# zfwangDP/X2-GNN

Measured on AMD Instinct MI355X. Metric: molecules/sec (fwd+bwd) on QM9 U0, batch=128, 1/2/4/8 MI355X, higher is better.
Workload: dtype fp32; 1 GPU; xgnn_poly U0 train step (config.json: L=4, D=128, H=16, sbf 7x6), S160, fwd+loss+bwd+allreduce+clip+Adam+EMA; per_gpu_batch=128, global_batch=128, line_nodes_per_gpu=21058, triplets_per_gpu=194060, parallelism=dp1, hip_graph=True

## Files before the change

include/x2g.h:

```cpp
#ifndef X2G_H
#define X2G_H

#include <stddef.h>
#include <stdint.h>

#ifdef __cplusplus
extern "C" {
#endif

#define X2G_OK 0
#define X2G_EINVAL 1001
#define X2G_EUNSUPPORTED 1002
#define X2G_EWORKSPACE 1003

#define X2G_EDGE_NONE 0
#define X2G_EDGE_PER_TRIPLET 1
#define X2G_EDGE_PER_DST 2

int x2g_abi_version(void);
const char* x2g_status_string(int status);


int x2g_csr_rowptr(const int32_t* keys, int64_t n, int64_t n_seg, int32_t* rowptr, void* stream);

// ... 230 lines not shown
int x2g_smooth_l1_mean_fwd_grad(const float* pred, const float* target, int64_t n, float beta, float* out,
                                float* dpred_unit, void* stream);


size_t x2g_linear_wgrad_workspace(int64_t rows, int32_t out_features, int32_t in_features);


#define X2G_ACCUM_WGRAD 1
#define X2G_DEFER_SLAB_SUM 2

typedef struct {
  const float* part_w;
  const float* part_b;
  float* dw;
  float* db;
  int64_t n_w;
  int32_t n_b;
  int32_t splits;
  int32_t ld;
  int32_t cols;
} x2g_slab_job;

int x2g_slab_sum_batch(const x2g_slab_job* jobs, int32_t njobs, int32_t accum, void* stream);

#define X2G_GATE_MAX_JOBS 8
typedef struct {
  const float* x;
  const float* w;
  const float* b;
  float* out;
  const float* g;
  float* dx;
  const float* dx_add;
  float* dw;
  float* db;
} x2g_gate_job;
int x2g_rbf_pool_fwd_batch(const x2g_gate_job* jobs, int32_t n_jobs, const float* rbf, const int32_t* rowptr,
                           int64_t n_seg, int32_t D, int32_t R, void* stream);
size_t x2g_rbf_gate_bwd_batch_workspace(int64_t rows, int32_t D, int32_t R, int32_t n_jobs);
int x2g_rbf_gate_bwd_batch(const x2g_gate_job* jobs, int32_t n_jobs, const int32_t* owner, const float* rbf,
                           int64_t rows, int32_t D, int32_t R, float* drbf, int flags, x2g_slab_job* slab_jobs,
                           void* workspace, size_t workspace_bytes, void* stream);

int32_t x2g_linear_wgrad_splits(int64_t rows, int32_t out_features, int32_t in_features);
int32_t x2g_dense_bwd_splits(int64_t rows, int32_t in_features, int32_t out_features);
int64_t x2g_dense_bwd_slab_offset(int64_t rows, int32_t in_features, int32_t out_features);

int x2g_linear_wgrad_ex(const float* dy, const float* x, int64_t rows, int32_t out_features,
                        int32_t in_features, float* dw, float* db, int flags, void* workspace,
                        size_t workspace_bytes, void* stream);

#define X2G_ACT_NONE 0
#define X2G_ACT_SILU 1

int x2g_dense_fwd(const float* x, const float* w, const float* b, int64_t rows, int32_t in_features,
                  int32_t out_features, int act, const float* res, float* y, float* z, void* stream);

size_t x2g_dense_bwd_workspace(int64_t rows, int32_t in_features, int32_t out_features);

int x2g_dense_bwd(const float* dy, const float* z, int act, const float* x, const float* w, int64_t rows,
                  int32_t in_features, int32_t out_features, float* dx, float* dw, float* db, void* workspace,
                  size_t workspace_bytes, void* stream);

int x2g_dense_bwd_ex(const float* dy, const float* z, int act, const float* x, const float* w, int64_t rows,
                     int32_t in_features, int32_t out_features, float* dx, const float* dx_add, float* dw,
                     float* db, int flags, void* workspace, size_t workspace_bytes, void* stream);

int x2g_residual_fwd(const float* x, const float* w0, const float* b0, const float* w1, const float* b1,
                     int64_t rows, int32_t dim, float* h, float* z0, float* z1, float* y, void* stream);

#define X2G_MAX_GROUPS 8

typedef struct {
  const float* x;
  const float* w;
  const float* b;
  const float* res;
  float* y;
  float* z;
} x2g_dense_fwd_group;

typedef struct {
  const float* dy;
  const float* z;
  const float* x;
  const float* w;
  float* dx;
  const float* dx_add;
  float* dw;
  float* db;
} x2g_dense_bwd_group;

int x2g_dense_fwd_batched(const x2g_dense_fwd_group* groups, int32_t num_groups, int64_t rows,
                          int32_t in_features, int32_t out_features, int act, void* stream);

int x2g_dense_bwd_batched(const x2g_dense_bwd_group* groups, int32_t num_groups, int64_t rows,
                          int32_t in_features, int32_t out_features, int act, int flags, void* workspace,
                          size_t workspace_bytes, void* stream);

typedef struct {
  const float* h;
  const float* w;
  const float* b;
  float* dh;
  float* dw;
  float* db;
} x2g_head_group;

int x2g_readout_head_fwd(const x2g_head_group* groups, int32_t num_groups, int64_t rows, int32_t dim, float* out,
                         void* stream);
size_t x2g_readout_head_bwd_workspace(int64_t rows, int32_t dim, int32_t num_groups);
int32_t x2g_readout_head_bwd_splits(int64_t rows);
int x2g_readout_head_bwd(const float* dout, const x2g_head_group* groups, int32_t num_groups, int64_t rows,
                         int32_t dim, int flags, void* workspace, size_t workspace_bytes, void* stream);

int x2g_readout_head_pool_fwd(const x2g_head_group* groups, int32_t num_groups, int64_t rows, int32_t dim,
                              const int32_t* seg_rowptr, int64_t num_segments, float* out_seg, void* stream);
int x2g_readout_head_pool_bwd(const float* dout_seg, const int32_t* seg_rowptr, int64_t num_segments,
                              const x2g_head_group* groups, int32_t num_groups, int64_t rows, int32_t dim, int flags,
                              void* workspace, size_t workspace_bytes, void* stream);


#define X2G_OPT_LR 0
#define X2G_OPT_BETA1 1
#define X2G_OPT_BETA2 2
#define X2G_OPT_EPS 3
#define X2G_OPT_MAX_NORM 4
#define X2G_OPT_EMA_DECAY 5
#define X2G_OPT_STEP 6
#define X2G_OPT_NORM 7
#define X2G_OPT_CLIP 8
#define X2G_OPT_STEP_SIZE 9
#define X2G_OPT_BC2_SQRT 10
#define X2G_OPT_WARMUP 11
#define X2G_OPT_DECAY_STEPS 12
#define X2G_OPT_DECAY_RATE 13
#define X2G_OPT_BASE_LR 14
#define X2G_OPT_STAIRCASE 15

size_t x2g_optimizer_workspace(int64_t n);

int x2g_clip_adam_ema(float* params, const float* grads, float* exp_avg, float* exp_avg_sq, float* ema,
                      int64_t n, float* scalars, void* workspace, size_t workspace_bytes, void* stream);
#define X2G_OPT_ZERO_GRADS 1
int x2g_clip_adam_ema_ex(float* params, float* grads, float* exp_avg, float* exp_avg_sq, float* ema, int64_t n,
                         float* scalars, int flags, void* workspace, size_t workspace_bytes, void* stream);

#define X2G_CHAIN_MAX_STAGES 8
#define X2G_CHAIN_SILU 1
#define X2G_CHAIN_HOLD 2
#define X2G_CHAIN_RES_HELD 4
#define X2G_CHAIN_RES_EXT 8
#define X2G_CHAIN_RES_ACCUM 16

typedef struct {
  const float* w;
  const float* b;
  float* z;
  float* y;
  float* wt;
  int32_t flags;
} x2g_chain_stage;

int x2g_chain_fwd(const float* x, const float* res_ext, const x2g_chain_stage* stages, int32_t n_stages,
                  int64_t rows, int32_t dim, float* in_t, void* stream);

int x2g_chain_fwd_ln(const float* x, const float* row_stats, const int32_t* seg_rowptr, int64_t num_segments,
                     float eps, float* x_norm, float* seg_mean, float* seg_rstd, const float* res_ext,
                     const x2g_chain_stage* stages, int32_t n_stages, int64_t rows, int32_t dim, float* in_t,
                     void* stream);

#define X2G_CHAIN_MAX_JOBS 8
typedef struct {
  const float* x;
  const float* res_ext;
  const x2g_chain_stage* stages;
  float* in_t;
} x2g_chain_fwd_job;
int x2g_chain_fwd_batch(const x2g_chain_fwd_job* jobs, int32_t num_jobs, int32_t n_stages, int64_t rows, int32_t dim,
                        void* stream);

int64_t x2g_chain_t_floats(int64_t rows, int32_t dim);

typedef struct {
  const float* w;
  const float* wt;
  const float* z;
  float* dz;
  int32_t flags;
} x2g_chain_bwd_stage;

int x2g_chain_bwd(const float* dy, const float* dy_add, const x2g_chain_bwd_stage* stages, int32_t n_stages,
                  int64_t rows, int32_t dim, float* dx, float* d_res_ext, float* dz_t, void* stream);
int x2g_chain_bwd_ln(const float* dy, const float* dy_add, const x2g_chain_bwd_stage* stages, int32_t n_stages,
                     int64_t rows, int32_t dim, float* dx, float* d_res_ext, float* dz_t, const float* x_norm,
                     float* row_gstats, void* stream);

typedef struct {
  const float* dy;
  const float* dy_add;
  const x2g_chain_bwd_stage* stages;
  float* dx;
  float* d_res_ext;
  float* dz_t;
} x2g_chain_bwd_job;
int x2g_chain_bwd_batch(const x2g_chain_bwd_job* jobs, int32_t num_jobs, int32_t n_stages, int64_t rows, int32_t dim,
                        void* stream);

size_t x2g_chain_wgrad_workspace(int64_t rows, int32_t dim, int32_t n_stages);
int x2g_chain_wgrad(const float* in_t, const float* dz_t, int32_t n_stages, int64_t rows, int32_t dim,
                    float* const* dw, float* const* db, int flags, void* workspace, size_t workspace_bytes,
                    void* stream);

typedef struct {
  const float* dy;
  const float* x;
  float* dw;
  float* db;
} x2g_wgrad_job;

size_t x2g_wgrad_batched_workspace(int64_t rows, int32_t dim, int32_t num_jobs);
int32_t x2g_wgrad_batched_splits(int64_t rows, int32_t dim, int32_t num_jobs);
int x2g_wgrad_batched(const x2g_wgrad_job* jobs, int32_t num_jobs, int64_t rows, int32_t dim, int flags,
                      void* workspace, size_t workspace_bytes, void* stream);

typedef struct {
  const float* w;
  const float* b;
  float* out;
  float* wt;
} x2g_proj;

int x2g_conv_proj_fwd(const float* x, const float* rbf, int32_t rbf_dim, const float* w_rbf, const x2g_proj* proj,
                      int64_t rows, int32_t dim, float* x_t, float* xs_t, void* stream);

typedef struct {
  const float* g;
  const float* w;
  const float* wt;
  float* g_t;
} x2g_proj_grad;

int32_t x2g_conv_proj_bwd_gate_splits(int64_t rows);
size_t x2g_conv_proj_bwd_gate_workspace(int64_t rows, int32_t rbf_dim);
int x2g_conv_proj_bwd_gate(const x2g_proj_grad* grads, int64_t rows, int32_t dim, const float* x, const float* rbf,
                           int32_t rbf_dim, const float* w_rbf, float* dx, const float* dx_add, float* drbf,
                           float* dw_rbf, int flags, void* workspace, size_t workspace_bytes, void* stream);

typedef struct {
  const float* dy_t;
  const float* x_t;
  float* dw;
  float* db;
  int32_t ld;
  int32_t cols;
} x2g_tiled_job;

#define X2G_TILED_MAX_JOBS 64
size_t x2g_tiled_wgrad_flat_workspace(int64_t rows, int32_t dim, int32_t num_jobs);
int x2g_tiled_wgrad_flat(const x2g_tiled_job* jobs, int32_t num_jobs, int64_t rows, int32_t dim, int flags,
                         x2g_slab_job* slab_jobs, void* workspace, size_t workspace_bytes, void* stream);
size_t x2g_tiled_wgrad_flat_rows_workspace(const int64_t* job_rows, int32_t num_jobs, int32_t dim);
int x2g_tiled_wgrad_flat_rows(const x2g_tiled_job* jobs, const int64_t* job_rows, int32_t num_jobs, int32_t dim,
                              int flags, x2g_slab_job* slab_jobs, void* workspace, size_t workspace_bytes,
                              void* stream);

size_t x2g_tiled_wgrad_workspace(int64_t rows, int32_t dim, int32_t num_jobs);
int x2g_tiled_wgrad(const x2g_tiled_job* jobs, int32_t num_jobs, int64_t rows, int32_t dim, int flags,
                    void* workspace, size_t workspace_bytes, void* stream);

#define X2G_TABLE_MAX_STAGES 8

typedef struct {
  const float* w;
  const float* b;
  int32_t parent;
  int32_t act;
  float* z;
  float* y;
} x2g_table_stage;

int x2g_table_chain_fwd(const float* x, int64_t rows, int32_t dim, const x2g_table_stage* stages, int32_t n_stages,
                        void* stream);

typedef struct {
  const float* w;
  const float* in;
  const float* z;
  const float* dy;
  float* dw;
  float* db;
  int32_t parent;
  int32_t act;
  int32_t accum;
} x2g_table_bwd_stage;

size_t x2g_table_chain_bwd_workspace(int32_t n_stages);
int x2g_table_chain_bwd_ex(const x2g_table_bwd_stage* stages, int32_t n_stages, int64_t rows, int32_t dim, float* dx,
                           void* workspace, size_t workspace_bytes, void* stream);

int x2g_feat_fwd(const float* x, const float* env, int64_t rows, int32_t in_dim, const float* w1, const float* b1,
                 const float* w2, const float* b2, float* y, float* xs_t, float* z1_t, float* y1_t, float* z2_t,
                 void* stream);

int x2g_feat_bwd(const float* dy, const float* z2_t, const float* z1_t, const float* w2, int64_t rows, float* dz2_t,
                 float* dz1_t, void* stream);

#ifdef __cplusplus
}
#endif

#endif
```

x2-gnn_amd/csrc/chain.hip:

```cpp
#include <math.h>

#include <type_traits>

#include "common.hpp"

namespace x2g {
namespace {

typedef float f4 __attribute__((ext_vector_type(4)));

constexpr int kCD = 128;
constexpr int kCWaves = 8;
constexpr int kCThreads = kCWaves * 64;

struct ChainFwdArgs {
  const float* x;
  const float* res;
  float* in_t;
  int64_t tf;
  int64_t R;
  int n;
  x2g_chain_stage st[X2G_CHAIN_MAX_STAGES];
};

// ... 378 lines not shown
  }
  float cnt = 0.f;
#pragma unroll
  for (int j = 0; j < kPW; ++j) cnt += (lane + 64 * j <= ln.G && pk[j] <= r0) ? 1.f : 0.f;
  for (int64_t k = lane + 64 * kPW; k <= ln.G; k += 64) cnt += ln.ptr[k] <= r0 ? 1.f : 0.f;
  const int64_t m0 = static_cast<int64_t>(wave64_sum(cnt)) - 1;
  auto ptr_at = [&](int64_t k) -> int {
    if (k >= 64 * kPW) return uniform(ln.ptr[k]);
    const int l = static_cast<int>(k & 63);
    switch (k >> 6) {
      case 0: return lane_bcast(pk[0], l);
      case 1: return lane_bcast(pk[1], l);
      case 2: return lane_bcast(pk[2], l);
      default: return lane_bcast(pk[3], l);
    }
  };
  constexpr int kSW = 4;
  for (int64_t m = m0 > 0 ? m0 : 0; m < ln.G; ++m) {
    const int p0 = ptr_at(m), p1 = ptr_at(m + 1);
    if (p0 >= r0 + nrows) break;
    if (p1 - p0 <= kLongMol) continue;
    const float n = static_cast<float>(p1 - p0);
    constexpr int kU = 4;
    float s = 0.f;
    for (int base = p0 + tid; base < p1; base += kU * kCThreads) {
      float v[kU];
#pragma unroll
      for (int u = 0; u < kU; ++u) {
        const int r = base + u * kCThreads;
        v[u] = r < p1 ? ln.stats[r].x : 0.f;
      }
#pragma unroll
      for (int u = 0; u < kU; ++u) s += v[u];
    }
    s = wave64_sum(s);
    if (lane == 0) red[w] = s;
    __syncthreads();
    float st = 0.f;
#pragma unroll
    for (int ww = 0; ww < kCWaves; ++ww) st += red[ww];
    const float mu = st / n;
    float q = 0.f;
    for (int base = p0 + tid; base < p1; base += kU * kCThreads) {
      float2 v[kU];
#pragma unroll
      for (int u = 0; u < kU; ++u) {
        const int r = base + u * kCThreads;
        v[u] = r < p1 ? ln.stats[r] : make_float2(mu, 0.f);
      }
#pragma unroll
      for (int u = 0; u < kU; ++u) {
        const float d = v[u].x - mu;
        q += fmaf(static_cast<float>(kCD) * d, d, v[u].y);
      }
    }
    q = wave64_sum(q);
    if (lane == 0) red[kCWaves + w] = q;
    __syncthreads();
    float qt = 0.f;
#pragma unroll
    for (int ww = 0; ww < kCWaves; ++ww) qt += red[kCWaves + ww];
    const float denom = sqrtf(qt / (n * static_cast<float>(kCD)) + ln.eps);
    const int lo = p0 > r0 ? p0 : r0, hi = p1 < r0 + nrows ? p1 : r0 + nrows;
    for (int r = lo + tid; r < hi; r += kCThreads) lnrow[r - r0] = make_float2(mu, denom);
    if (tid == 0 && p0 >= r0) {
      if (ln.mean) ln.mean[m] = mu;
      if (ln.rstd) ln.rstd[m] = 1.0f / denom;
    }
    __syncthreads();
  }
  for (int64_t m = (m0 > 0 ? m0 : 0) + w; m < ln.G; m += kCWaves) {
    const int p0 = ptr_at(m), p1 = ptr_at(m + 1);
    if (p0 >= r0 + nrows) break;
    if (p1 <= p0 || p1 - p0 > kLongMol) continue;
    const float n = static_cast<float>(p1 - p0);
    float2 sv[kSW];
#pragma unroll
    for (int j = 0; j < kSW; ++j) {
      const int r = p0 + lane + 64 * j;
      sv[j] = ln.stats[r < p1 ? r : p0];
    }
    float s = 0.f;
#pragma unroll
    for (int j = 0; j < kSW; ++j) s += p0 + lane + 64 * j < p1 ? sv[j].x : 0.f;
    for (int r = p0 + lane + 64 * kSW; r < p1; r += 64) s += ln.stats[r].x;
    const float mu = wave64_sum(s) / n;
    float q = 0.f;
#pragma unroll
    for (int j = 0; j < kSW; ++j) {
      const float d = sv[j].x - mu;
      q += p0 + lane + 64 * j < p1 ? fmaf(static_cast<float>(kCD) * d, d, sv[j].y) : 0.f;
    }
    for (int r = p0 + lane + 64 * kSW; r < p1; r += 64) {
      const float2 st = ln.stats[r];
      const float d = st.x - mu;
      q += fmaf(static_cast<float>(kCD) * d, d, st.y);
    }
    const float denom = sqrtf(wave64_sum(q) / (n * static_cast<float>(kCD)) + ln.eps);
    const int lo = p0 > r0 ? p0 : r0, hi = p1 < r0 + nrows ? p1 : r0 + nrows;
    for (int r = lo + lane; r < hi; r += 64) lnrow[r - r0] = make_float2(mu, denom);
    if (lane == 0 && p0 >= r0) {
      if (ln.mean) ln.mean[m] = mu;
      if (ln.rstd) ln.rstd[m] = 1.0f / denom;
    }
  }
  asm volatile("s_waitcnt vmcnt(0)" ::: "memory");
  __syncthreads();
#pragma unroll
  for (int u = 0; u < RB; ++u) {
    const int q = tid + kCThreads * u, r = q >> 5, c = q & 31;
    const bool ok = r < nrows;
    const float2 st = lnrow[ok ? r : 0];
    const f4 v = img[ipos(r, c)];
    f4 y;
#pragma unroll
    for (int e = 0; e < 4; ++e) y[e] = ok ? (v[e] - st.x) / st.y : 0.0f;
    img[ipos(r, c)] = y;
    if (ln.out && ok) *reinterpret_cast<f4*>(ln.out + (r0 + r) * kCD + 4 * c) = y;
  }
}

template <bool LN, int RB = kV2RB, bool TC = true>
__device__ __forceinline__ void chain_fwd_v4_run(const ChainFwdArgs& a, const ChainLn& ln) {
  static_assert(RB == 6 || RB == 3, "thirds of 2 or 1 row blocks");
  __shared__ f4 img0[RB * 16 * 32];
  __shared__ f4 img1[RB * 16 * 32];
  __shared__ f4 imgr[RB * 16 * 32];
  __shared__ float2 lnrow[LN ? RB * 16 : 1];
  __shared__ float lnred[LN ? 2 * kCWaves : 1];
  const int tid = threadIdx.x, lane = tid & 63, w = tid >> 6;
  const int rl = lane & 15, g = lane >> 4;
  const int64_t nblk = (a.R + 15) / 16, G = gridDim.x;
  const int64_t nch = (nblk + RB * G - 1) / (RB * G) * G;
  const int n = a.n;
  for (int64_t i = static_cast<int64_t>(blockIdx.x) * kCThreads + tid; i < static_cast<int64_t>(n) * kCD * kCD;
       i += G * kCThreads) {
    const int s = static_cast<int>(i / (kCD * kCD)), e = static_cast<int>(i % (kCD * kCD));
    if (a.st[s].wt) a.st[s].wt[e] = a.st[s].w[(e % kCD) * kCD + e / kCD];
  }
  for (int64_t ch = blockIdx.x; ch < nch; ch += G) {
    int r0, nrows;
    chunk_rows(ch, nch, nblk, a.R, r0, nrows);
    __syncthreads();
    if (LN)
      stage_rows_ln<RB>(img0, a.x, a.R, ln, lnrow, lnred, r0, nrows);
    else
      stage_rows<RB>(img0, a.x, nullptr, r0, nrows);
    if (a.res) stage_rows<RB>(imgr, a.res, nullptr, r0, nrows);
    f4 A[8], held[RB];
    load_slice<false>(a.st[0].w, w, rl, g, A);
#pragma unroll
    for (int rb = 0; rb < RB; ++rb) held[rb] = zero4();
    __syncthreads();
    if (a.in_t) {
      f4 xs[RB];
#pragma unroll
      for (int rb = 0; rb < RB; ++rb) xs[rb] = img0[ipos(16 * rb + rl, 4 * w + g)];
      store_t_slice(a.in_t, xs, r0, nrows, w, rl, g);
    }
    for (int s = 0; s < n; s += 2) {
      fwd4_stage<RB, TC>(a, s, img0, img1, imgr, A, held, r0, nrows, w, rl, g);
      if (s + 1 < n) fwd4_stage<RB, TC>(a, s + 1, img1, img0, imgr, A, held, r0, nrows, w, rl, g);
    }
  }
}

__global__ void __launch_bounds__(kCThreads, 1) chain_fwd_v4(const ChainFwdArgs a) { chain_fwd_v4_run<false>(a, {}); }

struct ChainFwdLnArgs {
  ChainFwdArgs a;
  ChainLn ln;
};
__global__ void __launch_bounds__(kCThreads, 1) chain_fwd_v4_ln(const ChainFwdLnArgs b) {
  chain_fwd_v4_run<true>(b.a, b.ln);
}
__global__ void __launch_bounds__(kCThreads, 1) chain_fwd_v4_ln_infer(const ChainFwdLnArgs b) {
  chain_fwd_v4_run<true, kV2RB, false>(b.a, b.ln);
}

constexpr int kChainMaxJobs = X2G_CHAIN_MAX_JOBS;
struct ChainFwdBatch {
  ChainFwdArgs a[kChainMaxJobs];
};
template <int RB>
__global__ void __launch_bounds__(kCThreads, 1) chain_fwd_v4_batch(const ChainFwdBatch b) {
  chain_fwd_v4_run<false, RB>(b.a[blockIdx.y], {});
}

template <int RB0, int RB1, int N>
__device__ __forceinline__ void bwd_elem(f4 (&gs)[N], f4 (&dh)[N], const f4 (&zc)[N], const f4 (&acc)[N],
                                         float hold_m, float held_m, float silu_m, float dres_acc_m, rsrc_t dres_r,
                                         rsrc_t dz_r, rsrc_t t_r, f4* __restrict__ out, int r0, int nrows, int w,
                                         int rl, int g) {
  const int col = 16 * w + 4 * g;
  const int j = rl & 3, m = rl >> 2, f = 16 * w + 4 * g + j;
  const int ntile = (nrows + 15) >> 4;
#pragma unroll
  for (int rb = RB0; rb < RB1; ++rb) {
    const int r = 16 * rb + rl;
    const int off = r < nrows ? 4 * ((r0 + r) * kCD + col) : kOOB;
    const f4 gv = acc[rb] + dh[rb] * hold_m;
    dh[rb] = dh[rb] * (1.0f - hold_m) + gv * held_m;
    if (dres_acc_m != 0.0f) {
      bstore4(dres_r, gv + bload4(dres_r, off, 0), off);
    } else {
      bstore4(dres_r, gv, off);
    }
    f4 dz;
#pragma unroll
    for (int e = 0; e < 4; ++e) dz[e] = gv[e] * (silu_m * silu_grad_fast(zc[rb][e]) + (1.0f - silu_m));
    bstore4(dz_r, dz, off);
    out[ipos(r, 4 * w + g)] = dz;
    gs[rb] = dz;
    f4 t = quad_transpose(dz, j);
#pragma unroll
    for (int e = 0; e < 4; ++e) t[e] = 16 * rb + 4 * m + e < nrows ? t[e] : 0.0f;
    bstore4(t_r, t, rb < ntile ? 4 * static_cast<int>((static_cast<int64_t>(r0 >> 4) + rb) * (16 * kCD) + f * 16 + 4 * m)
                               : kOOB);
  }
}

template <int RB = kV2RB>
__device__ __forceinline__ void store_img_lnstats(float* __restrict__ P, const f4* __restrict__ img,
                                                  const f4* __restrict__ yimg, float2* __restrict__ gs, int r0,
                                                  int nrows) {
  const int tid = threadIdx.x;
#pragma unroll
  for (int u = 0; u < RB; ++u) {
    const int q = tid + kCThreads * u, r = q >> 5, c = q & 31;
    const f4 g = img[ipos(r, c)], y = yimg[ipos(r, c)];
    if (r < nrows) *reinterpret_cast<f4*>(P + (r0 + r) * kCD + 4 * c) = g;
    const float s1 = half32_sum_hi((g[0] + g[1]) + (g[2] + g[3]));
    const float s2 = half32_sum_hi(fmaf(g[0], y[0], fmaf(g[1], y[1], fmaf(g[2], y[2], g[3] * y[3]))));
    if (c == 16 && r < nrows) gs[r0 + r] = make_float2(s1, s2);
  }
}

template <int RB = kV2RB>
__device__ __forceinline__ void chain_bwd_v3_run(const ChainBwdArgs& a) {
  static_assert(RB == 6 || RB == 3, "thirds of 2 or 1 row blocks");
  constexpr int BPT = RB / 3;
  __shared__ f4 img[2][RB * 16 * 32];
  __shared__ f4 yimg[RB * 16 * 32];
  const int tid = threadIdx.x, lane = tid & 63, w = tid >> 6;
  const int rl = lane & 15, g = lane >> 4;
  const int64_t nblk = (a.R + 15) / 16, G = gridDim.x;
  const int64_t nch = (nblk + RB * G - 1) / (RB * G) * G;
  const int n = a.n;
  const int col = 16 * w + 4 * g;
  for (int64_t ch = blockIdx.x; ch < nch; ch += G) {
    int r0, nrows;
    chunk_rows(ch, nch, nblk, a.R, r0, nrows);
    f4 A[8], dh[RB], zc[RB], gs[RB];
    auto load_z = [&](int s) {
      const rsrc_t zr = rsrc((a.st[s].flags & X2G_CHAIN_SILU) ? a.st[s].z : a.dy);
#pragma unroll
      for (int rb = 0; rb < RB; ++rb) {
        const int r = 16 * rb + rl;
        zc[rb] = bload4(zr, 4 * ((r0 + (r < nrows ? r : 0)) * kCD + col), 0);
      }
    };
    auto load_wslice = [&](int s, f4 (&dst)[8]) {
      if (a.st[s].wt)
        load_slice<false>(a.st[s].wt, w, rl, g, dst);
      else
        load_slice<true>(a.st[s].w, w, rl, g, dst);
    };
    auto elem_args = [&](int s, float& held_m, float& silu_m, float& dres_acc_m, rsrc_t& dres_r, rsrc_t& dz_r,
                         rsrc_t& t_r) {
      const x2g_chain_bwd_stage& S = a.st[s];
      const int fl = S.flags;
      held_m = (fl & X2G_CHAIN_RES_HELD) ? 1.0f : 0.0f;
      silu_m = (fl & X2G_CHAIN_SILU) ? 1.0f : 0.0f;
      const bool dres_on = (fl & X2G_CHAIN_RES_EXT) && a.dres;
      dres_acc_m = (fl & X2G_CHAIN_RES_ACCUM) ? 1.0f : 0.0f;
      dres_r = rsrc_n(dres_on ? a.dres : a.dy, a.R * kCD * 4, dres_on);
      dz_r = rsrc_n(S.dz ? S.dz : a.dy, a.R * kCD * 4, S.dz != nullptr);
      t_r = rsrc_n(a.dz_t ? a.dz_t + s * a.tf : a.dy, a.tf * 4, a.dz_t != nullptr);
    };
    if (a.ln_y) stage_rows_async<RB>(yimg, a.ln_y, a.R, r0);
    load_wslice(n - 1, A);
    load_z(n - 1);
    f4 acc0[RB];
    {
      const rsrc_t yr = rsrc(a.dy), ar = rsrc(a.dy_add ? a.dy_add : a.dy);
      const float am = a.dy_add ? 1.0f : 0.0f;
#pragma unroll
      for (int rb = 0; rb < RB; ++rb) {
        const int r = 16 * rb + rl;
        const int vo = 4 * ((r0 + (r < nrows ? r : 0)) * kCD + col);
        acc0[rb] = bload4(yr, vo, 0) + bload4(ar, vo, 0) * am;
        dh[rb] = zero4();
      }
    }
    int p = 0;
    __syncthreads();
    {
      float held_m, silu_m, dres_acc_m;
      rsrc_t dres_r, dz_r, t_r;
      elem_args(n - 1, held_m, silu_m, dres_acc_m, dres_r, dz_r, t_r);
      bwd_elem<0, RB>(gs, dh, zc, acc0, 0.0f, held_m, silu_m, dres_acc_m, dres_r, dz_r, t_r, img[p], r0, nrows,
                              w, rl, g);
    }
    __syncthreads();
    for (int s = n - 1; s >= 0; --s) {
      f4 An[8];
      load_wslice(s > 0 ? s - 1 : n - 1, An);
// ... 77 lines not shown
  const int tid = threadIdx.x, q = tid & 31;
#pragma unroll
  for (int u = 0; u < 4; ++u) {
    const int r = (tid >> 5) + 8 * u;
    *reinterpret_cast<f4*>(T + r * 128 + 4 * (q ^ (r & 15))) = v[u];
  }
}

__global__ void __launch_bounds__(kWThreads, 2) wgrad_batched_kernel(const WgradArgs a) {
  __shared__ __attribute__((aligned(16))) float Ds[2][32 * 128];
  __shared__ __attribute__((aligned(16))) float Xs[2][32 * 128];
  const int j = blockIdx.y;
  const x2g_wgrad_job& J = a.job[j];
  const int tid = threadIdx.x, lane = tid & 63, wave = tid >> 6, h = lane >> 5, i = lane & 31;
  const int nb = 32 * wave;
  const int64_t r0 = static_cast<int64_t>(blockIdx.x) * a.chunk_rows;
  const int64_t r1 = r0 + a.chunk_rows < a.R ? r0 + a.chunk_rows : a.R;
  floatx16 acc[4];
#pragma unroll
  for (int m = 0; m < 4; ++m)
#pragma unroll
    for (int e = 0; e < 16; ++e) acc[m][e] = 0.f;
  float bsum = 0.f;
  f4 vd[4], vx[4];
  int buf = 0;
  if (r0 < r1) {
    wtile_load(J.dy, r0, r1, vd);
    wtile_load(J.x, r0, r1, vx);
  }
  for (int64_t t = r0; t < r1; t += 32) {
    wtile_store(Ds[buf], vd);
    wtile_store(Xs[buf], vx);
    __syncthreads();
    if (t + 32 < r1) {
      wtile_load(J.dy, t + 32, r1, vd);
      wtile_load(J.x, t + 32, r1, vx);
    }
    const float* D = Ds[buf];
    const float* X = Xs[buf];
#pragma unroll
    for (int sg = 0; sg < 2; ++sg) {
#pragma unroll
      for (int s = 0; s < 8; ++s) {
        const int r = 16 * sg + s + 8 * h;
        const float av = D[wswz(r, nb + i)];
#pragma unroll
        for (int m = 0; m < 4; ++m) acc[m] = __builtin_amdgcn_mfma_f32_32x32x2f32(av, X[wswz(r, 32 * m + i)], acc[m], 0, 0, 0);
      }
    }
    if (J.db && tid < 128) {
#pragma unroll 8
      for (int rr = 0; rr < 32; ++rr) bsum += D[wswz(rr, tid)];
    }
    buf ^= 1;
  }
  float* slab = a.part_w[j] + static_cast<int64_t>(blockIdx.x) * kCD * kCD;
#pragma unroll
  for (int m = 0; m < 4; ++m)
#pragma unroll
    for (int e = 0; e < 16; ++e) slab[(nb + (e & 3) + 8 * (e >> 2) + 4 * h) * kCD + 32 * m + i] = acc[m][e];
  if (J.db && tid < 128) a.part_b[j][static_cast<int64_t>(blockIdx.x) * kCD + tid] = bsum;
}

constexpr int kWTiles = 2;

__device__ __forceinline__ int tpos(int f, int q) { return f * 4 + (q ^ (((f >> 3) & 1) * 3)); }

struct ChainWgradArgs {
  const float* in_t[X2G_CHAIN_MAX_STAGES];
  const float* dz_t[X2G_CHAIN_MAX_STAGES];
  int64_t ntiles;
  float* part_w[X2G_CHAIN_MAX_STAGES];
  float* part_b[X2G_CHAIN_MAX_STAGES];
  int has_b[X2G_CHAIN_MAX_STAGES];
  int splits;
};

template <int NB, bool SPREAD = true, int WT = kWTiles>
__device__ __forceinline__ void tiled_segment(const float* __restrict__ dz, const float* __restrict__ xin, int64_t t0,
                                              int64_t t1, bool has_b, float* __restrict__ slab,
                                              float* __restrict__ slab_b, f4 (*Ds)[WT][512],
                                              f4 (*Xs)[WT][512]) {
  const int tid = threadIdx.x, lane = tid & 63, w = tid >> 6;
  const int rl = lane & 15, g = lane >> 4;
  const int nsteps = static_cast<int>((t1 - t0 + WT - 1) / WT);
  const int P = 64 * w + lane;
  const int src_chunk = (P >> 2) * 4 + ((P & 3) ^ (((P >> 5) & 1) * 3));
  auto issue = [&](int step) {
    const int b = step % NB;
#pragma unroll
    for (int k = 0; k < WT; ++k) {
      int64_t t = t0 + static_cast<int64_t>(step) * WT + k;
      t = t < t1 ? t : t0;
      __builtin_amdgcn_global_load_lds(dz + t * 2048 + 4 * src_chunk, &Ds[b][k][64 * w], 16, 0, 0);
      __builtin_amdgcn_global_load_lds(xin + t * 2048 + 4 * src_chunk, &Xs[b][k][64 * w], 16, 0, 0);
    }
  };
  f4 acc[8];
#pragma unroll
  for (int bk = 0; bk < 8; ++bk) acc[bk] = zero4();
  float bsum = 0.f;
#pragma unroll
  for (int p = 0; p < NB - 1; ++p)
    if (p < nsteps) issue(p);
  for (int i = 0; i < nsteps; ++i) {
    const int ahead = nsteps - 1 - i < NB - 2 ? nsteps - 1 - i : NB - 2;
    if (ahead >= 2)
      asm volatile("s_waitcnt vmcnt(%0)" ::"n"(4 * WT) : "memory");
    else if (ahead == 1)
      asm volatile("s_waitcnt vmcnt(%0)" ::"n"(2 * WT) : "memory");
    else
      asm volatile("s_waitcnt vmcnt(0)" ::: "memory");
    asm volatile("s_waitcnt lgkmcnt(0)" ::: "memory");
    __builtin_amdgcn_s_barrier();
    if (i + NB - 1 < nsteps) issue(i + NB - 1);
    const int b = i % NB;
#pragma unroll
    for (int k = 0; k < WT; ++k) {
      if (t0 + static_cast<int64_t>(i) * WT + k >= t1) break;
      const f4 av = Ds[b][k][tpos(16 * w + rl, g)];
      f4 bv[8];
#pragma unroll
      for (int bk = 0; bk < 8; ++bk) bv[bk] = Xs[b][k][tpos(16 * bk + rl, g)];
#pragma unroll
      for (int e = 0; e < 4; ++e)
#pragma unroll
        for (int bk = 0; bk < 8; ++bk) acc[bk] = __builtin_amdgcn_mfma_f32_16x16x4f32(av[e], bv[bk][e], acc[bk], 0, 0, 0);
      if (SPREAD && has_b) {
        const f4 v = Ds[b][k][tpos(tid & (kCD - 1), tid >> 7)];
        bsum += (v[0] + v[1]) + (v[2] + v[3]);
      }
      if (!SPREAD && tid < 128) {
#pragma unroll
        for (int q = 0; q < 4; ++q) {
          const f4 v = Ds[b][k][tpos(tid, q)];
          bsum += (v[0] + v[1]) + (v[2] + v[3]);
        }
      }
    }
  }
#pragma unroll
  for (int bk = 0; bk < 8; ++bk)
#pragma unroll
    for (int e = 0; e < 4; ++e) slab[(16 * w + 4 * g + e) * kCD + 16 * bk + rl] = acc[bk][e];
  if (!SPREAD && has_b && tid < 128) slab_b[tid] = bsum;
  if (SPREAD && has_b) {
    __shared__ float bred[4 * kCD];
    bred[tid] = bsum;
    __syncthreads();
    if (tid < kCD) slab_b[tid] = ((bred[tid] + bred[kCD + tid]) + bred[2 * kCD + tid]) + bred[3 * kCD + tid];
  }
}

template <bool SPREAD, int WT>
__device__ __forceinline__ void tiled_segment2(const float* __restrict__ dz, const float* __restrict__ xin, int64_t t0,
                                               int64_t t1, bool has_b, float* __restrict__ slab,
                                               float* __restrict__ slab_b, f4 (*D0)[512], f4 (*X0)[512],
                                               f4 (*D1)[512], f4 (*X1)[512]) {
  const int tid = threadIdx.x, lane = tid & 63, w = tid >> 6;
  const int rl = lane & 15, g = lane >> 4;
  const int nsteps = static_cast<int>((t1 - t0 + WT - 1) / WT);
  const int P = 64 * w + lane;
  const int src_chunk = (P >> 2) * 4 + ((P & 3) ^ (((P >> 5) & 1) * 3));
  const int64_t nt = t1 - t0;
  const int nbytes = static_cast<int>(nt * 8192 < 0x7fffffff ? nt * 8192 : 0x7fffffff);
  const rsrc_t dr = __builtin_amdgcn_make_buffer_rsrc(const_cast<float*>(dz + t0 * 2048), static_cast<short>(0), nbytes,
                                                      0x00020000);
  const rsrc_t xr = __builtin_amdgcn_make_buffer_rsrc(const_cast<float*>(xin + t0 * 2048), static_cast<short>(0), nbytes,
                                                      0x00020000);
  auto issue = [&](int step, f4 (*Dd)[512], f4 (*Xd)[512]) {
#pragma unroll
    for (int k = 0; k < WT; ++k) {
      int tt = step * WT + k;
      tt = tt < nt ? tt : 0;
      const int vo = tt * 8192 + 16 * src_chunk;
      __builtin_amdgcn_raw_ptr_buffer_load_lds(dr, (__attribute__((address_space(3))) void*)(&Dd[k][64 * w]), 16, vo, 0,
                                               0, 0);
      __builtin_amdgcn_raw_ptr_buffer_load_lds(xr, (__attribute__((address_space(3))) void*)(&Xd[k][64 * w]), 16, vo, 0,
                                               0, 0);
    }
  };
  f4 acc[8];
#pragma unroll
  for (int bk = 0; bk < 8; ++bk) acc[bk] = zero4();
  float bsum = 0.f;
  auto body = [&](int i, f4 (*Dc)[512], f4 (*Xc)[512], f4 (*Dn)[512], f4 (*Xn)[512]) {
    asm volatile("s_waitcnt vmcnt(0)" ::: "memory");
    asm volatile("s_waitcnt lgkmcnt(0)" ::: "memory");
    __builtin_amdgcn_s_barrier();
    issue(i + 1, Dn, Xn);
#pragma unroll
    for (int k = 0; k < WT; ++k) {
      if (t0 + static_cast<int64_t>(i) * WT + k >= t1) break;
      const f4 av = Dc[k][tpos(16 * w + rl, g)];
      f4 bv[8];
#pragma unroll
      for (int bk = 0; bk < 8; ++bk) bv[bk] = Xc[k][tpos(16 * bk + rl, g)];
#pragma unroll
      for (int e = 0; e < 4; ++e)
#pragma unroll
        for (int bk = 0; bk < 8; ++bk) acc[bk] = __builtin_amdgcn_mfma_f32_16x16x4f32(av[e], bv[bk][e], acc[bk], 0, 0, 0);
      if (SPREAD && has_b) {
        const f4 v = Dc[k][tpos(tid & (kCD - 1), tid >> 7)];
        bsum += (v[0] + v[1]) + (v[2] + v[3]);
      }
      if (!SPREAD && tid < 128) {
#pragma unroll
        for (int q = 0; q < 4; ++q) {
          const f4 v = Dc[k][tpos(tid, q)];
          bsum += (v[0] + v[1]) + (v[2] + v[3]);
        }
      }
    }
  };
  if (nsteps > 0) issue(0, D0, X0);
  for (int i = 0; i < nsteps; i += 2) {
    body(i, D0, X0, D1, X1);
    if (i + 1 >= nsteps) break;
    body(i + 1, D1, X1, D0, X0);
  }
  asm volatile("s_waitcnt vmcnt(0)" ::: "memory");
#pragma unroll
  for (int bk = 0; bk < 8; ++bk)
#pragma unroll
    for (int e = 0; e < 4; ++e) slab[(16 * w + 4 * g + e) * kCD + 16 * bk + rl] = acc[bk][e];
  if (!SPREAD && has_b && tid < 128) slab_b[tid] = bsum;
  if (SPREAD && has_b) {
    __shared__ float bred[4 * kCD];
    bred[tid] = bsum;
    __syncthreads();
    if (tid < kCD) slab_b[tid] = ((bred[tid] + bred[kCD + tid]) + bred[2 * kCD + tid]) + bred[3 * kCD + tid];
  }
}

__global__ void __launch_bounds__(kCThreads, 1) chain_wgrad_kernel(const ChainWgradArgs a) {
  __shared__ f4 Ds[3][kWTiles][512];
  __shared__ f4 Xs[3][kWTiles][512];
  const int s = blockIdx.y, c = blockIdx.x;
  const int64_t t0 = c * a.ntiles / a.splits, t1 = (c + 1) * a.ntiles / a.splits;
  tiled_segment<3>(a.dz_t[s], a.in_t[s], t0, t1, a.has_b[s] != 0, a.part_w[s] + static_cast<int64_t>(c) * kCD * kCD,
                a.part_b[s] + static_cast<int64_t>(c) * kCD, Ds, Xs);
}

struct TiledFlatArgs {
  const float* in_t[X2G_TILED_MAX_JOBS];
  const float* dz_t[X2G_TILED_MAX_JOBS];
  float* slab_w[X2G_TILED_MAX_JOBS];
  float* slab_b[X2G_TILED_MAX_JOBS];
  int wg_lo[X2G_TILED_MAX_JOBS];
  int has_b[X2G_TILED_MAX_JOBS];
  int64_t tile0[X2G_TILED_MAX_JOBS + 1];
  int64_t total;
  int njobs;
};

template <int NB, bool SPREAD = true, int WT = kWTiles, int WPC = 1>
__global__ void __launch_bounds__(kCThreads, 2 * WPC) tiled_flat_kernel(const TiledFlatArgs a) {
  static_assert(NB == 2, "the flat launch's two named buffers (tiled_segment2)");
  __shared__ f4 D0[WT][512];
  __shared__ f4 X0[WT][512];
  __shared__ f4 D1[WT][512];
  __shared__ f4 X1[WT][512];
  const int64_t G = gridDim.x, i = blockIdx.x;
  const int64_t lo = i * a.total / G, hi = (i + 1) * a.total / G;
  int j0 = 0;
  while (j0 < a.njobs && a.tile0[j0 + 1] <= lo) ++j0;
  for (int j = j0; j < a.njobs && a.tile0[j] < hi; ++j) {
    const int64_t s0 = lo > a.tile0[j] ? lo : a.tile0[j];
    const int64_t s1 = hi < a.tile0[j + 1] ? hi : a.tile0[j + 1];
    if (s0 >= s1) continue;
    __syncthreads();
    const int64_t k = i - a.wg_lo[j];
    tiled_segment2<SPREAD, WT>(a.dz_t[j], a.in_t[j], s0 - a.tile0[j], s1 - a.tile0[j], a.has_b[j] != 0,
                               a.slab_w[j] + k * kCD * kCD, a.slab_b[j] + k * kCD, D0, X0, D1, X1);
  }
}

inline int chain_wgrad_splits_of(int64_t ntiles, int stages) {
  int64_t per = 256 / stages;
  const int64_t cap = (ntiles + 3) / 4;
  if (per > cap) per = cap;
  return static_cast<int>(per < 1 ? 1 : per);
}

constexpr int kRbfMax = 8;
constexpr int kGateRB = 3;

struct ProjFwdArgs {
  const float* x;
  const float* rbf;
  const float* wr;
  int RR;
  x2g_proj p[4];
  float* x_t;
  float* xs_t;
  int64_t R;
};

template <int RB>
__device__ __forceinline__ void load_rows_slice(const float* P, int r0, int nrows, int w, int rl, int g,
                                                f4 (&v)[RB]) {
  const rsrc_t pr = rsrc(P);
#pragma unroll
  for (int rb = 0; rb < RB; ++rb) {
    const int r = 16 * rb + rl;
    const bool ok = r < nrows;
    v[rb] = bload4(pr, 4 * ((r0 + (ok ? r : 0)) * kCD + 16 * w + 4 * g), 0) * (ok ? 1.0f : 0.0f);
  }
}

template <int NJ, int RB = kV2RB, int NT = kCThreads>
__device__ __forceinline__ void stage_rbf(float* __restrict__ srbf, const float* __restrict__ rbf, int RR, int r0,
                                          int nrows) {
  for (int i = threadIdx.x; i < RB * 16 * NJ; i += NT) {
    const int r = i / NJ, j = i % NJ;
    srbf[i] = (r < nrows && j < RR) ? rbf[static_cast<int64_t>(r0 + r) * RR + j] : 0.0f;
  }
}

template <int NJ>
__device__ __forceinline__ f4 gate_filter(const float* __restrict__ srbf, const float* __restrict__ swr, int r, int c0) {
  f4 f;
#pragma unroll
  for (int e = 0; e < 4; ++e) {
    float acc = 0.0f;
#pragma unroll
    for (int j = 0; j < NJ; ++j) acc = fmaf(swr[(c0 + e) * NJ + j], srbf[r * NJ + j], acc);
    f[e] = acc;
  }
  return f;
}

template <int NJ>
__global__ void __launch_bounds__(kCThreads, 2) conv_proj_fwd_kernel(const ProjFwdArgs a) {
  constexpr int RB = kV2RB;
  __shared__ f4 img[2][RB * 16 * 32];
  __shared__ float srbf[RB * 16 * NJ];
  __shared__ float swr[kCD * NJ];
  const int tid = threadIdx.x, lane = tid & 63, w = tid >> 6;
  const int rl = lane & 15, g = lane >> 4;
  const int64_t nblk = (a.R + 15) / 16, G = gridDim.x;
  const int64_t nch = (nblk + RB * G - 1) / (RB * G) * G;
  for (int i = tid; i < kCD * NJ; i += kCThreads) {
    const int c = i / NJ, j = i % NJ;
    swr[i] = j < a.RR ? a.wr[c * a.RR + j] : 0.0f;
  }
  for (int64_t i = static_cast<int64_t>(blockIdx.x) * kCThreads + tid; i < 4 * kCD * kCD; i += G * kCThreads) {
    const int p = static_cast<int>(i / (kCD * kCD)), e = static_cast<int>(i % (kCD * kCD));
    if (a.p[p].wt) a.p[p].wt[e] = a.p[p].w[(e % kCD) * kCD + e / kCD];
  }
  for (int64_t ch = blockIdx.x; ch < nch; ch += G) {
    int r0, nrows;
    chunk_rows(ch, nch, nblk, a.R, r0, nrows);
    __syncthreads();
    stage_rows<RB>(img[0], a.x, nullptr, r0, nrows);
    stage_rbf<NJ, RB>(srbf, a.rbf, a.RR, r0, nrows);
    f4 A[8];
    load_slice<false>(a.p[0].w, w, rl, g, A);
    __syncthreads();
    {
      f4 xv[RB], xs[RB];
#pragma unroll
      for (int rb = 0; rb < RB; ++rb) {
        const int r = 16 * rb + rl;
        xv[rb] = img[0][ipos(r, 4 * w + g)];
        xs[rb] = xv[rb] * gate_filter<NJ>(srbf, swr, r, 16 * w + 4 * g);
        img[1][ipos(r, 4 * w + g)] = xs[rb];
      }
      if (a.x_t) store_t_slice(a.x_t, xv, r0, nrows, w, rl, g);
      if (a.xs_t) store_t_slice(a.xs_t, xs, r0, nrows, w, rl, g);
    }
    __syncthreads();
#pragma unroll 1
    for (int p = 0; p < 4; ++p) {
      const x2g_proj& P = a.p[p];
      f4 An[8];
      load_slice<false>(a.p[p + 1 < 4 ? p + 1 : 0].w, w, rl, g, An);
      const f4 bias = bload4(rsrc(P.b ? P.b : P.w), 4 * (16 * w + 4 * g), 0) * (P.b ? 1.0f : 0.0f);
      f4 acc[RB];
      slice_gemm(img[(p == 1 || p == 2) ? 1 : 0], A, acc, rl, g);
#pragma unroll
      for (int rb = 0; rb < RB; ++rb) {
        const int r = 16 * rb + rl;
        if (r < nrows) *reinterpret_cast<f4*>(P.out + (r0 + r) * kCD + 16 * w + 4 * g) = acc[rb] + bias;
      }
      pin(An);
#pragma unroll
      for (int b = 0; b < 8; ++b) A[b] = An[b];
    }
  }
}

struct ProjBwdGateArgs {
  x2g_proj_grad gr[4];
  const float* dx_add;
  float* dx;
  const float* x;
  const float* rbf;
  const float* wr;
  float* drbf;
  float* part_w;
  int RR;
  int drbf_acc;
  int64_t R;
};


template <int NJ, bool TW>
__global__ void __launch_bounds__(kCThreads, 2) conv_proj_bwd_gate_kernel(const ProjBwdGateArgs a) {
  constexpr int RB = kGateRB;
  constexpr int kImg = RB * 16 * 32;
  __shared__ f4 img_k[kImg], img_v[kImg];
  __shared__ f4 img_q[kImg], img_s[kImg];
  __shared__ float srbf[RB * 16 * NJ];
  __shared__ float swr[kCD * NJ];
  __shared__ float red[kCWaves * RB * 16 * 16];
  __shared__ float sdw[kCD * NJ];
  const int tid = threadIdx.x, lane = tid & 63, w = tid >> 6;
  const int rl = lane & 15, g = lane >> 4;
  const int64_t nblk = (a.R + 15) / 16, G = gridDim.x;
  const int64_t nch = (nblk + RB * G - 1) / (RB * G) * G;
  const int nk = static_cast<int>(nch / G);
  const int c0 = 16 * w + 4 * g;
  for (int i = tid; i < kCD * NJ; i += kCThreads) {
    const int c = i / NJ, j = i % NJ;
    swr[i] = j < a.RR ? a.wr[c * a.RR + j] : 0.0f;
    sdw[i] = 0.0f;
  }
  auto load_ws = [&](int p, f4 (&dst)[8]) {
    if (TW)
      load_slice<false>(a.gr[p].wt, w, rl, g, dst);
    else
      load_slice<true>(a.gr[p].w, w, rl, g, dst);
  };
  auto t_copy = [&](int p, const f4* im, int r0, int nrows) {
    f4 v[RB];
#pragma unroll
    for (int rb = 0; rb < RB; ++rb) v[rb] = im[ipos(16 * rb + rl, 4 * w + g)];
    store_t_slice(a.gr[p].g_t, v, r0, nrows, w, rl, g);
  };
  auto chunk = [&](int k, int& r0, int& nrows) { chunk_rows(blockIdx.x + k * G, nch, nblk, a.R, r0, nrows); };
  const int64_t bytes = a.R * kCD * 4;
  const rsrc_t ar = rsrc_n(a.dx_add, bytes, a.dx_add != nullptr);
  const rsrc_t dr = rsrc_n(a.dx, bytes, true);
  const rsrc_t xr = rsrc_n(a.x, bytes, true);
  const rsrc_t rr = rsrc_n(a.rbf, a.R * a.RR * 4, true);
  const rsrc_t br = rsrc_n(a.drbf, a.R * a.RR * 4, a.drbf != nullptr);
  const rsrc_t bo = rsrc_n(a.drbf, a.R * a.RR * 4, a.drbf != nullptr && a.drbf_acc);
  static_assert(RB * 16 * NJ <= kCThreads && RB * 16 * kRbfMax <= kCThreads, "one srbf / drbf element per thread");
  constexpr int kWL = TW ? 8 : 32;
  constexpr int kKVWait = 3 * RB + 2 * kWL < 63 ? 3 * RB + 2 * kWL : 63;
  constexpr int kQSWait = 2 * RB + 2 * kWL < 63 ? 2 * RB + 2 * kWL : 63;
  if (nk > 0) {
    int r0, nrows;
    chunk(0, r0, nrows);
    stage_rows_async<RB>(img_k, a.gr[1].g, a.R, r0);
    stage_rows_async<RB>(img_v, a.gr[2].g, a.R, r0);
  }
  f4 A[8], An[8];
  load_ws(1, A);
  load_ws(2, An);
  __syncthreads();
  float dold = 0.0f;
  int doff = kOOB;
  auto drbf_out = [&]() {
    const int i = doff == kOOB ? 0 : tid, r = i / a.RR, j = i % a.RR;
    float sum = 0.0f;
#pragma unroll
    for (int ww = 0; ww < kCWaves; ++ww) sum += red[(ww * RB * 16 + r) * 16 + j];
    __builtin_amdgcn_raw_buffer_store_b32(__builtin_bit_cast(unsigned, dold + sum), br, doff, 0, 0);
  };
  for (int k = 0; k < nk; ++k) {
    int r0, nrows;
    chunk(k, r0, nrows);
    if (k > 0)
      asm volatile("s_waitcnt vmcnt(%0)" ::"n"(kKVWait) : "memory");
    else
      asm volatile("s_waitcnt vmcnt(0)" ::: "memory");
    __syncthreads();
    drbf_out();
    stage_rows_async<RB>(img_q, a.gr[0].g, a.R, r0);
    stage_rows_async<RB>(img_s, a.gr[3].g, a.R, r0);
    asm volatile("" ::: "memory");
    f4 xv[RB];
#pragma unroll
    for (int rb = 0; rb < RB; ++rb) {
      const int r = 16 * rb + rl;
      xv[rb] = bload4(xr, 4 * ((r0 + (r < nrows ? r : 0)) * kCD + c0), 0);
    }
    float rbv;
    {
      const int r = tid / NJ, j = tid % NJ;
      rbv = bload1(rr, (tid < RB * 16 * NJ && r < nrows && j < a.RR) ? 4 * ((r0 + r) * a.RR + j) : kOOB, 0);
    }
    t_copy(1, img_k, r0, nrows);
    t_copy(2, img_v, r0, nrows);
    f4 acc1[RB];
    slice_gemm(img_k, A, acc1, rl, g);
    load_ws(0, A);
    slice_gemm<RB, false>(img_v, An, acc1, rl, g);
    load_ws(3, An);
    if (tid < RB * 16 * NJ) srbf[tid] = rbv;
    asm volatile("s_waitcnt vmcnt(%0)" ::"n"(kQSWait) : "memory");
    __syncthreads();
    doff = tid < nrows * a.RR ? 4 * (r0 * a.RR + tid) : kOOB;
    dold = bload1(bo, doff, 0);
    f4 xa[RB];
#pragma unroll
    for (int rb = 0; rb < RB; ++rb) {
      const int r = 16 * rb + rl;
      xa[rb] = bload4(ar, 4 * ((r0 + (r < nrows ? r : 0)) * kCD + c0), 0);
    }
    {
      const bool more = k + 1 < nk;
      int r1, n1;
      chunk(more ? k + 1 : k, r1, n1);
      stage_rows_async<RB>(img_k, a.gr[1].g, a.R, r1, more);
      stage_rows_async<RB>(img_v, a.gr[2].g, a.R, r1, more);
      asm volatile("" ::: "memory");
    }
    t_copy(0, img_q, r0, nrows);
    t_copy(3, img_s, r0, nrows);
    f4 acc[RB], d1[RB];
    slice_gemm(img_q, A, acc, rl, g);
    load_ws(1, A);
    f4 wrv;
#pragma unroll
    for (int e = 0; e < 4; ++e) wrv[e] = swr[(c0 + e) * NJ + (rl < NJ ? rl : 0)] * (rl < NJ ? 1.0f : 0.0f);
    float aw[4][NJ];
#pragma unroll
    for (int i = 0; i < 4; ++i)
#pragma unroll
      for (int j = 0; j < NJ; ++j) aw[i][j] = 0.0f;
#pragma unroll
    for (int rb = 0; rb < RB; ++rb) {
      const int r = 16 * rb + rl;
      d1[rb] = xa[rb] + acc1[rb] * gate_filter<NJ>(srbf, swr, r, c0);
      const f4 df = r < nrows ? acc1[rb] * xv[rb] : zero4();
#pragma unroll
      for (int i = 0; i < 4; ++i)
#pragma unroll
        for (int j = 0; j < NJ; ++j) aw[i][j] = fmaf(df[i], srbf[r * NJ + j], aw[i][j]);
      f4 pd = zero4();
#pragma unroll
      for (int e = 0; e < 4; ++e) pd = __builtin_amdgcn_mfma_f32_16x16x4f32(df[e], wrv[e], pd, 0, 0, 0);
#pragma unroll
      for (int i = 0; i < 4; ++i) red[(w * RB * 16 + 16 * rb + 4 * g + i) * 16 + rl] = pd[i];
    }
#pragma unroll
    for (int i = 0; i < 4; ++i)
#pragma unroll
      for (int j = 0; j < NJ; ++j) sdw[(c0 + i) * NJ + j] += row_sum16(aw[i][j]);
    slice_gemm<RB, false>(img_s, An, acc, rl, g);
    load_ws(2, An);
#pragma unroll
    for (int rb = 0; rb < RB; ++rb) {
      const int r = 16 * rb + rl;
      bstore4(dr, d1[rb] + acc[rb], r < nrows ? 4 * ((r0 + r) * kCD + c0) : kOOB);
    }
  }
  __syncthreads();
  drbf_out();
  float* slab = a.part_w + static_cast<int64_t>(blockIdx.x) * kCD * a.RR;
  for (int i = tid; i < kCD * a.RR; i += kCThreads) slab[i] = sdw[(i / a.RR) * NJ + i % a.RR];
}

inline bool al16(const void* p) { return reinterpret_cast<uintptr_t>(p) % 16 == 0; }

inline int wgrad_chunk_rows(int64_t R, int jobs) {
  const int64_t target = 512;
  const int64_t per_job = (target + jobs - 1) / jobs;
  int64_t cr = (R + per_job - 1) / per_job;
  cr = (cr + 31) / 32 * 32;
  return static_cast<int>(cr < 64 ? 64 : cr);
}

}
}

using namespace x2g;

X2G_API int64_t x2g_chain_t_floats(int64_t rows, int32_t dim) {
  return rows > 0 && dim > 0 ? (rows + 15) / 16 * 16 * dim : 0;
}

static int chain_fwd_prepare(const float* x, const float* res_ext, const x2g_chain_stage* stages, int32_t n_stages,
                             int64_t rows, int32_t dim, float* in_t, ChainFwdArgs& a, bool& empty) {
  empty = false;
  if (!stages || n_stages < 1 || n_stages > X2G_CHAIN_MAX_STAGES || rows < 0 || dim <= 0) return X2G_EINVAL;
  if (dim != kCD || rows * kCD * 4 >= (int64_t(1) << 31)) return X2G_EUNSUPPORTED;
  a = ChainFwdArgs{};
  a.x = x;
  a.res = res_ext;
  a.in_t = in_t;
  a.tf = x2g_chain_t_floats(rows, dim);
  a.R = rows;
  a.n = n_stages;
  int n_ext = 0, held = 0;
  for (int s = 0; s < n_stages; ++s) {
    const x2g_chain_stage& S = stages[s];
    if (!S.w || (s == n_stages - 1 && !S.y)) return X2G_EINVAL;
    if (S.flags & ~(X2G_CHAIN_SILU | X2G_CHAIN_HOLD | X2G_CHAIN_RES_HELD | X2G_CHAIN_RES_EXT)) return X2G_EINVAL;
    if ((S.flags & X2G_CHAIN_RES_EXT) && (S.flags & (X2G_CHAIN_HOLD | X2G_CHAIN_RES_HELD))) return X2G_EINVAL;
    if (S.flags & X2G_CHAIN_RES_EXT) held = 0;
    if (S.flags & X2G_CHAIN_HOLD) held = 1;
    if ((S.flags & X2G_CHAIN_RES_HELD) && !held) return X2G_EINVAL;
    if (S.flags & X2G_CHAIN_RES_EXT) ++n_ext;
    if (!al16(S.w) || !al16(S.b) || !al16(S.z) || !al16(S.y) || !al16(S.wt)) return X2G_EUNSUPPORTED;
    a.st[s] = S;
  }
  if (n_ext > 1 || (n_ext && !res_ext)) return X2G_EINVAL;
  if (rows == 0) {
    empty = true;
    return X2G_OK;
  }
  if (!x) return X2G_EINVAL;
  if (!al16(x) || !al16(res_ext) || !al16(in_t)) return X2G_EUNSUPPORTED;
  return X2G_OK;
}

X2G_API int x2g_chain_fwd(const float* x, const float* res_ext, const x2g_chain_stage* stages, int32_t n_stages,
                          int64_t rows, int32_t dim, float* in_t, void* stream) {
  ChainFwdArgs a{};
  bool empty;
  if (int rc = chain_fwd_prepare(x, res_ext, stages, n_stages, rows, dim, in_t, a, empty)) return rc;
  if (empty) return X2G_OK;
  hipStream_t st = as_stream(stream);
  const int64_t nblk = (rows + 15) / 16;
  chain_fwd_v4<<<static_cast<unsigned>(nblk < 256 ? nblk : 256), kCThreads, 0, st>>>(a);
  return last_launch_status();
}

X2G_API int x2g_chain_fwd_ln(const float* x, const float* row_stats, const int32_t* seg_rowptr, int64_t num_segments,
                             float eps, float* x_norm, float* seg_mean, float* seg_rstd, const float* res_ext,
                             const x2g_chain_stage* stages, int32_t n_stages, int64_t rows, int32_t dim, float* in_t,
                             void* stream) {
  ChainFwdArgs a{};
  bool empty;
  if (int rc = chain_fwd_prepare(x, res_ext, stages, n_stages, rows, dim, in_t, a, empty)) return rc;
  if (num_segments < 0 || (rows > 0 && (!row_stats || !seg_rowptr || num_segments < 1))) return X2G_EINVAL;
  if (reinterpret_cast<uintptr_t>(row_stats) % 8 || !al16(x_norm)) return X2G_EUNSUPPORTED;
  if (empty) return X2G_OK;
  const ChainFwdLnArgs b{a, {reinterpret_cast<const float2*>(row_stats), seg_rowptr, x_norm, seg_mean, seg_rstd,
                             num_segments, eps}};
  const int64_t nblk = (rows + 15) / 16;
  bool infer = b.a.in_t == nullptr;
  for (int s = 0; s < b.a.n; ++s) infer = infer && b.a.st[s].z == nullptr;
  if (infer)
    chain_fwd_v4_ln_infer<<<static_cast<unsigned>(nblk < 256 ? nblk : 256), kCThreads, 0, as_stream(stream)>>>(b);
  else
    chain_fwd_v4_ln<<<static_cast<unsigned>(nblk < 256 ? nblk : 256), kCThreads, 0, as_stream(stream)>>>(b);
  return last_launch_status();
}

static int chain_bwd_prepare(const float* dy, const float* dy_add, const x2g_chain_bwd_stage* stages, int32_t n_stages,
                             int64_t rows, int32_t dim, float* dx, float* d_res_ext, float* dz_t, ChainBwdArgs& a,
                             bool& empty, bool& res_accum) {
  empty = false;
  res_accum = false;
  if (!stages || n_stages < 1 || n_stages > X2G_CHAIN_MAX_STAGES || rows < 0 || dim <= 0) return X2G_EINVAL;
  if (dim != kCD || rows * kCD * 4 >= (int64_t(1) << 31)) return X2G_EUNSUPPORTED;
  a = ChainBwdArgs{};
  a.dy = dy;
  a.dy_add = dy_add;
  a.dx = dx;
  a.dres = d_res_ext;
  a.dz_t = dz_t;
  a.tf = x2g_chain_t_floats(rows, dim);
  a.R = rows;
  a.n = n_stages;
  int n_ext = 0, held = 0;
  for (int s = 0; s < n_stages; ++s) {
    const x2g_chain_bwd_stage& S = stages[s];
    if (!S.w || ((S.flags & X2G_CHAIN_SILU) && !S.z)) return X2G_EINVAL;
    if (S.flags & ~(X2G_CHAIN_SILU | X2G_CHAIN_HOLD | X2G_CHAIN_RES_HELD | X2G_CHAIN_RES_EXT | X2G_CHAIN_RES_ACCUM))
      return X2G_EINVAL;
    if ((S.flags & X2G_CHAIN_RES_ACCUM) && !(S.flags & X2G_CHAIN_RES_EXT)) return X2G_EINVAL;
    if ((S.flags & X2G_CHAIN_RES_EXT) && (S.flags & (X2G_CHAIN_HOLD | X2G_CHAIN_RES_HELD))) return X2G_EINVAL;
    if (S.flags & X2G_CHAIN_RES_EXT) held = 0;
    if (S.flags & X2G_CHAIN_HOLD) held = 1;
    if ((S.flags & X2G_CHAIN_RES_HELD) && !held) return X2G_EINVAL;
    if (S.flags & X2G_CHAIN_RES_EXT) ++n_ext;
    if (S.flags & X2G_CHAIN_RES_ACCUM) res_accum = true;
    if (!al16(S.w) || !al16(S.wt) || !al16(S.z) || !al16(S.dz)) return X2G_EUNSUPPORTED;
    a.st[s] = S;
  }
  if (n_ext > 1) return X2G_EINVAL;
  if (rows == 0) {
    empty = true;
    return X2G_OK;
  }
  if (!dy || !dx) return X2G_EINVAL;
  if (!al16(dy) || !al16(dy_add) || !al16(dx) || !al16(d_res_ext) || !al16(dz_t)) return X2G_EUNSUPPORTED;
  return X2G_OK;
}

static int chain_bwd_launch(const ChainBwdArgs& a, int64_t rows, void* stream) {
  hipStream_t st = as_stream(stream);
  {
    const int64_t nblk = (rows + 15) / 16;
    ChainBwdBatch b{};
    b.a[0] = a;
    const dim3 grid(static_cast<unsigned>(nblk < 256 ? nblk : 256), 1);
    chain_bwd_v3_batch<kV2RB><<<grid, kCThreads, 0, st>>>(b);
  }
  return last_launch_status();
}

X2G_API int x2g_chain_bwd_ln(const float* dy, const float* dy_add, const x2g_chain_bwd_stage* stages,
                             int32_t n_stages, int64_t rows, int32_t dim, float* dx, float* d_res_ext, float* dz_t,
                             const float* x_norm, float* row_gstats, void* stream) {
  ChainBwdArgs a{};
  bool empty, res_accum;
  if (int rc = chain_bwd_prepare(dy, dy_add, stages, n_stages, rows, dim, dx, d_res_ext, dz_t, a, empty, res_accum))
    return rc;
  if (rows > 0 && (!x_norm || !row_gstats)) return X2G_EINVAL;
  if (!al16(x_norm) || reinterpret_cast<uintptr_t>(row_gstats) % 8) return X2G_EUNSUPPORTED;
  if (empty) return X2G_OK;
  a.ln_y = x_norm;
  a.ln_gstats = reinterpret_cast<float2*>(row_gstats);
  return chain_bwd_launch(a, rows, stream);
}

X2G_API int x2g_chain_bwd(const float* dy, const float* dy_add, const x2g_chain_bwd_stage* stages, int32_t n_stages,
                          int64_t rows, int32_t dim, float* dx, float* d_res_ext, float* dz_t, void* stream) {
  ChainBwdArgs a{};
  bool empty, res_accum;
  if (int rc = chain_bwd_prepare(dy, dy_add, stages, n_stages, rows, dim, dx, d_res_ext, dz_t, a, empty, res_accum))
    return rc;
  if (empty) return X2G_OK;
  return chain_bwd_launch(a, rows, stream);
}

static inline unsigned chain_batch_grid(int64_t rows, int n_jobs) {
  const int64_t nblk = (rows + 15) / 16, per = 256 / n_jobs;
  return static_cast<unsigned>(nblk < per ? nblk : (per < 1 ? 1 : per));
}

static inline bool chain_batch_rb3(int64_t rows, unsigned grid_x) {
  const int64_t nblk = (rows + 15) / 16;
  return nblk <= 3 * static_cast<int64_t>(grid_x);
}

X2G_API int x2g_chain_fwd_batch(const x2g_chain_fwd_job* jobs, int32_t n_jobs, int32_t n_stages, int64_t rows,
                                int32_t dim, void* stream) {
  if (!jobs || n_jobs < 1 || n_jobs > kChainMaxJobs) return X2G_EINVAL;
  ChainFwdBatch b{};
  bool empty = false;
  for (int j = 0; j < n_jobs; ++j) {
    const x2g_chain_fwd_job& J = jobs[j];
    if (int rc = chain_fwd_prepare(J.x, J.res_ext, J.stages, n_stages, rows, dim, J.in_t, b.a[j], empty)) return rc;
  }
  if (empty) return X2G_OK;
  const dim3 grid(chain_batch_grid(rows, n_jobs), static_cast<unsigned>(n_jobs));
  if (chain_batch_rb3(rows, grid.x))
// ... 39 lines not shown
  if (!jobs || num_jobs < 1 || num_jobs > X2G_CHAIN_MAX_STAGES || rows <= 0 || dim <= 0 ||
      (flags & ~(X2G_ACCUM_WGRAD | X2G_DEFER_SLAB_SUM)))
    return X2G_EINVAL;
  if (dim != kCD || rows * kCD * 4 >= (int64_t(1) << 31)) return X2G_EUNSUPPORTED;
  const size_t need = x2g_wgrad_batched_workspace(rows, dim, num_jobs);
  if (!workspace || workspace_bytes < need) return X2G_EWORKSPACE;
  WgradArgs a{};
  a.R = rows;
  a.chunk_rows = wgrad_chunk_rows(rows, num_jobs);
  const int splits = x2g_wgrad_batched_splits(rows, dim, num_jobs);
  const size_t per_job = need / num_jobs;
  x2g_slab_job sj[X2G_CHAIN_MAX_STAGES];
  for (int j = 0; j < num_jobs; ++j) {
    const x2g_wgrad_job& J = jobs[j];
    if (!J.dy || !J.x || !J.dw) return X2G_EINVAL;
    if (!al16(J.dy) || !al16(J.x)) return X2G_EUNSUPPORTED;
    a.job[j] = J;
    a.part_w[j] = reinterpret_cast<float*>(static_cast<char*>(workspace) + per_job * j);
    a.part_b[j] = a.part_w[j] + static_cast<int64_t>(splits) * kCD * kCD;
    sj[j] = x2g_slab_job{a.part_w[j], J.db ? a.part_b[j] : nullptr, J.dw, J.db, kCD * kCD, J.db ? kCD : 0, splits};
  }
  hipStream_t st = as_stream(stream);
  wgrad_batched_kernel<<<dim3(static_cast<unsigned>(splits), static_cast<unsigned>(num_jobs)), kWThreads, 0, st>>>(a);
  const int rc = last_launch_status();
  if (rc || (flags & X2G_DEFER_SLAB_SUM)) return rc;
  return x2g_slab_sum_batch(sj, num_jobs, (flags & X2G_ACCUM_WGRAD) ? 1 : 0, stream);
}

static int32_t chain_wgrad_splits(int64_t rows, int32_t dim, int32_t n_stages) {
  if (rows <= 0 || dim != kCD || n_stages < 1 || n_stages > X2G_CHAIN_MAX_STAGES) return 0;
  return chain_wgrad_splits_of((rows + 15) / 16, n_stages);
}

X2G_API size_t x2g_chain_wgrad_workspace(int64_t rows, int32_t dim, int32_t n_stages) {
  const int32_t splits = chain_wgrad_splits(rows, dim, n_stages);
  return static_cast<size_t>(splits > 0 ? n_stages : 0) * splits * (kCD * kCD + kCD) * sizeof(float);
}

X2G_API int x2g_chain_wgrad(const float* in_t, const float* dz_t, int32_t n_stages, int64_t rows, int32_t dim,
                            float* const* dw, float* const* db, int flags, void* workspace, size_t workspace_bytes,
                            void* stream) {
  if (!in_t || !dz_t || !dw || n_stages < 1 || n_stages > X2G_CHAIN_MAX_STAGES || rows <= 0 || dim <= 0 ||
      (flags & ~(X2G_ACCUM_WGRAD | X2G_DEFER_SLAB_SUM)))
    return X2G_EINVAL;
  if (dim != kCD || rows * kCD * 4 >= (int64_t(1) << 31)) return X2G_EUNSUPPORTED;
  if (!al16(in_t) || !al16(dz_t)) return X2G_EUNSUPPORTED;
  const size_t need = x2g_chain_wgrad_workspace(rows, dim, n_stages);
  if (!workspace || workspace_bytes < need) return X2G_EWORKSPACE;
  ChainWgradArgs a{};
  const int64_t tf = x2g_chain_t_floats(rows, dim);
  for (int j = 0; j < n_stages; ++j) {
    a.in_t[j] = in_t + j * tf;
    a.dz_t[j] = dz_t + j * tf;
  }
  a.ntiles = (rows + 15) / 16;
  a.splits = chain_wgrad_splits(rows, dim, n_stages);
  const size_t per = need / n_stages;
  x2g_slab_job sj[X2G_CHAIN_MAX_STAGES];
  for (int j = 0; j < n_stages; ++j) {
    if (!dw[j]) return X2G_EINVAL;
    const bool hb = db && db[j];
    a.part_w[j] = reinterpret_cast<float*>(static_cast<char*>(workspace) + per * j);
    a.part_b[j] = a.part_w[j] + static_cast<int64_t>(a.splits) * kCD * kCD;
    a.has_b[j] = hb;
    sj[j] = x2g_slab_job{a.part_w[j], hb ? a.part_b[j] : nullptr, dw[j], hb ? db[j] : nullptr, kCD * kCD,
                         hb ? kCD : 0, a.splits};
  }
  chain_wgrad_kernel<<<dim3(static_cast<unsigned>(a.splits), static_cast<unsigned>(n_stages)), kCThreads, 0,
                       as_stream(stream)>>>(a);
  const int rc = last_launch_status();
  if (rc || (flags & X2G_DEFER_SLAB_SUM)) return rc;
  return x2g_slab_sum_batch(sj, n_stages, (flags & X2G_ACCUM_WGRAD) ? 1 : 0, stream);
}

static inline unsigned v2_grid(int64_t rows) {
  const int64_t nblk = (rows + 15) / 16;
  return static_cast<unsigned>(nblk < 256 ? nblk : 256);
}

static inline unsigned proj_grid(int64_t rows) {
  const int64_t nblk = (rows + 15) / 16, cap = 256;
  return static_cast<unsigned>(nblk < cap ? nblk : cap);
}

X2G_API int x2g_conv_proj_fwd(const float* x, const float* rbf, int32_t rbf_dim, const float* w_rbf,
                              const x2g_proj* proj, int64_t rows, int32_t dim, float* x_t, float* xs_t, void* stream) {
  if (!proj || rows < 0 || dim <= 0 || rbf_dim <= 0) return X2G_EINVAL;
  if (dim != kCD || rbf_dim > kRbfMax || rows * kCD * 4 >= (int64_t(1) << 31)) return X2G_EUNSUPPORTED;
  if (rows == 0) return X2G_OK;
  if (!x || !rbf || !w_rbf) return X2G_EINVAL;
  ProjFwdArgs a{};
  a.x = x;
  a.rbf = rbf;
  a.wr = w_rbf;
  a.RR = rbf_dim;
  a.x_t = x_t;
  a.xs_t = xs_t;
  a.R = rows;
  for (int p = 0; p < 4; ++p) {
    if (!proj[p].w || !proj[p].out) return X2G_EINVAL;
    if (!al16(proj[p].w) || !al16(proj[p].b) || !al16(proj[p].out) || !al16(proj[p].wt)) return X2G_EUNSUPPORTED;
    a.p[p] = proj[p];
  }
  if (!al16(x) || !al16(x_t) || !al16(xs_t)) return X2G_EUNSUPPORTED;
  if (rbf_dim <= 6)
    conv_proj_fwd_kernel<6><<<proj_grid(rows), kCThreads, 0, as_stream(stream)>>>(a);
  else
    conv_proj_fwd_kernel<8><<<proj_grid(rows), kCThreads, 0, as_stream(stream)>>>(a);
  return last_launch_status();
}

X2G_API int32_t x2g_conv_proj_bwd_gate_splits(int64_t rows) { return rows > 0 ? static_cast<int32_t>(proj_grid(rows)) : 0; }

X2G_API size_t x2g_conv_proj_bwd_gate_workspace(int64_t rows, int32_t rbf_dim) {
  if (rows <= 0 || rbf_dim <= 0) return 0;
  return static_cast<size_t>(proj_grid(rows)) * kCD * rbf_dim * sizeof(float);
}

X2G_API int x2g_conv_proj_bwd_gate(const x2g_proj_grad* grads, int64_t rows, int32_t dim, const float* x,
                                   const float* rbf, int32_t rbf_dim, const float* w_rbf, float* dx,
                                   const float* dx_add, float* drbf, float* dw_rbf, int flags, void* ws, size_t wsb,
                                   void* stream) {
  if (!grads || rows < 0 || dim <= 0 || rbf_dim <= 0 || !dw_rbf) return X2G_EINVAL;
  if (flags & ~(X2G_ACCUM_WGRAD | X2G_DEFER_SLAB_SUM | X2G_GATE_DRBF_ACCUM)) return X2G_EINVAL;
  if (dim != kCD || rbf_dim > kRbfMax || rows * kCD * 4 >= (int64_t(1) << 31)) return X2G_EUNSUPPORTED;
  hipStream_t st = as_stream(stream);
  if (rows == 0) {
    if (flags & X2G_DEFER_SLAB_SUM) return X2G_EINVAL;
    if (flags & X2G_ACCUM_WGRAD) return X2G_OK;
    const hipError_t e = hipMemsetAsync(dw_rbf, 0, sizeof(float) * kCD * rbf_dim, st);
    return e == hipSuccess ? X2G_OK : static_cast<int>(e);
  }
  if (!dx || !x || !rbf || !w_rbf) return X2G_EINVAL;
  if (!ws || wsb < x2g_conv_proj_bwd_gate_workspace(rows, rbf_dim)) return X2G_EWORKSPACE;
  ProjBwdGateArgs a{};
  for (int p = 0; p < 4; ++p) {
    if (!grads[p].g || !grads[p].w) return X2G_EINVAL;
    if (!al16(grads[p].g) || !al16(grads[p].w) || !al16(grads[p].wt) || !al16(grads[p].g_t)) return X2G_EUNSUPPORTED;
    a.gr[p] = grads[p];
  }
  if (!al16(dx) || !al16(dx_add) || !al16(x)) return X2G_EUNSUPPORTED;
  a.dx_add = dx_add;
  a.dx = dx;
  a.x = x;
  a.rbf = rbf;
  a.wr = w_rbf;
  a.drbf = drbf;
  a.part_w = static_cast<float*>(ws);
  a.RR = rbf_dim;
  a.drbf_acc = (flags & X2G_GATE_DRBF_ACCUM) ? 1 : 0;
  a.R = rows;
  const unsigned grid = proj_grid(rows);
  const bool tw = grads[0].wt && grads[1].wt && grads[2].wt && grads[3].wt;
  if (rbf_dim <= 6) {
    if (tw)
      conv_proj_bwd_gate_kernel<6, true><<<grid, kCThreads, 0, st>>>(a);
    else
      conv_proj_bwd_gate_kernel<6, false><<<grid, kCThreads, 0, st>>>(a);
  } else if (tw) {
    conv_proj_bwd_gate_kernel<8, true><<<grid, kCThreads, 0, st>>>(a);
  } else {
    conv_proj_bwd_gate_kernel<8, false><<<grid, kCThreads, 0, st>>>(a);
  }
  const int rc = last_launch_status();
  if (rc || (flags & X2G_DEFER_SLAB_SUM)) return rc;
  x2g_slab_job sj{a.part_w, nullptr, dw_rbf, nullptr, static_cast<int64_t>(kCD) * rbf_dim, 0,
                  static_cast<int32_t>(grid), 0, 0};
  return x2g_slab_sum_batch(&sj, 1, (flags & X2G_ACCUM_WGRAD) ? 1 : 0, stream);
}

constexpr int kFlatWPC = 2;
static inline unsigned flat_grid(int64_t total) {
  const int64_t cap = 256 * kFlatWPC;
  return static_cast<unsigned>(total < cap ? (total < 1 ? 1 : total) : cap);
}

static inline void flat_span(int64_t t0, int64_t t1, int64_t total, int64_t G, int& lo, int& n) {
  auto owner = [&](int64_t t) {
    int64_t i = (t * G) / total;
    while (i + 1 < G && (i + 1) * total / G <= t) ++i;
    while (i > 0 && i * total / G > t) --i;
    return static_cast<int>(i);
  };
  lo = owner(t0);
  n = owner(t1 - 1) - lo + 1;
}

static inline bool flat_tiles(const int64_t* rows, int num_jobs, int64_t* tile0) {
  tile0[0] = 0;
  for (int j = 0; j < num_jobs; ++j) {
    if (rows[j] <= 0 || rows[j] * kCD * 4 >= (int64_t(1) << 31)) return false;
    tile0[j + 1] = tile0[j] + (rows[j] + 15) / 16;
  }
  return true;
}

static size_t flat_workspace(const int64_t* rows, int32_t num_jobs, int32_t dim) {
  if (!rows || dim != kCD || num_jobs < 1 || num_jobs > X2G_TILED_MAX_JOBS) return 0;
  int64_t tile0[X2G_TILED_MAX_JOBS + 1];
  if (!flat_tiles(rows, num_jobs, tile0)) return 0;
  const int64_t total = tile0[num_jobs], G = flat_grid(total);
  int64_t slabs = 0;
  for (int j = 0; j < num_jobs; ++j) {
    int lo, n;
    flat_span(tile0[j], tile0[j + 1], total, G, lo, n);
    slabs += n;
  }
  return static_cast<size_t>(slabs) * (kCD * kCD + kCD) * sizeof(float);
}

static int flat_launch(const x2g_tiled_job* jobs, const int64_t* rows, int32_t num_jobs, int32_t dim, int flags,
                       x2g_slab_job* slab_jobs, void* workspace, size_t workspace_bytes, void* stream) {
  if (!jobs || !rows || num_jobs < 1 || num_jobs > X2G_TILED_MAX_JOBS || dim <= 0 ||
      (flags & ~(X2G_ACCUM_WGRAD | X2G_DEFER_SLAB_SUM)))
    return X2G_EINVAL;
  for (int j = 0; j < num_jobs; ++j)
    if (rows[j] <= 0) return X2G_EINVAL;
  if (dim != kCD) return X2G_EUNSUPPORTED;
  if ((flags & X2G_DEFER_SLAB_SUM) && !slab_jobs) return X2G_EINVAL;
  TiledFlatArgs a{};
  if (!flat_tiles(rows, num_jobs, a.tile0)) return X2G_EUNSUPPORTED;
  const size_t need = flat_workspace(rows, num_jobs, dim);
  if (!workspace || workspace_bytes < need) return X2G_EWORKSPACE;
  a.total = a.tile0[num_jobs];
  a.njobs = num_jobs;
  const int64_t G = flat_grid(a.total);
  x2g_slab_job sj[X2G_TILED_MAX_JOBS];
  float* base = static_cast<float*>(workspace);
  for (int j = 0; j < num_jobs; ++j) {
    const x2g_tiled_job& J = jobs[j];
    if (!J.dy_t || !J.x_t || !J.dw) return X2G_EINVAL;
    if (!al16(J.dy_t) || !al16(J.x_t)) return X2G_EUNSUPPORTED;
    if (J.ld < 0 || (J.ld > 0 && (J.cols < 1 || J.cols > kCD || J.cols > J.ld))) return X2G_EINVAL;
    int lo, n;
    flat_span(a.tile0[j], a.tile0[j + 1], a.total, G, lo, n);
    a.in_t[j] = J.x_t;
    a.dz_t[j] = J.dy_t;
    a.wg_lo[j] = lo;
    a.has_b[j] = J.db != nullptr;
    a.slab_w[j] = base;
    a.slab_b[j] = base + static_cast<int64_t>(n) * kCD * kCD;
    base += static_cast<int64_t>(n) * (kCD * kCD + kCD);
    sj[j] = x2g_slab_job{a.slab_w[j], J.db ? a.slab_b[j] : nullptr, J.dw, J.db, kCD * kCD, J.db ? kCD : 0, n,
                         J.ld, J.cols};
  }
  tiled_flat_kernel<2, true, 2, kFlatWPC><<<static_cast<unsigned>(G), kCThreads, 0, as_stream(stream)>>>(a);
  const int rc = last_launch_status();
  if (rc) return rc;
  if (flags & X2G_DEFER_SLAB_SUM) {
    for (int j = 0; j < num_jobs; ++j) slab_jobs[j] = sj[j];
    return X2G_OK;
  }
  return x2g_slab_sum_batch(sj, num_jobs, (flags & X2G_ACCUM_WGRAD) ? 1 : 0, stream);
}

X2G_API size_t x2g_tiled_wgrad_flat_workspace(int64_t rows, int32_t dim, int32_t num_jobs) {
  if (rows <= 0 || num_jobs < 1 || num_jobs > X2G_TILED_MAX_JOBS) return 0;
  int64_t r[X2G_TILED_MAX_JOBS];
  for (int j = 0; j < num_jobs; ++j) r[j] = rows;
  return flat_workspace(r, num_jobs, dim);
}

X2G_API int x2g_tiled_wgrad_flat(const x2g_tiled_job* jobs, int32_t num_jobs, int64_t rows, int32_t dim, int flags,
                                 x2g_slab_job* slab_jobs, void* workspace, size_t workspace_bytes, void* stream) {
  if (rows <= 0 || num_jobs < 1 || num_jobs > X2G_TILED_MAX_JOBS) return X2G_EINVAL;
  int64_t r[X2G_TILED_MAX_JOBS];
  for (int j = 0; j < num_jobs; ++j) r[j] = rows;
  return flat_launch(jobs, r, num_jobs, dim, flags, slab_jobs, workspace, workspace_bytes, stream);
}

X2G_API size_t x2g_tiled_wgrad_flat_rows_workspace(const int64_t* job_rows, int32_t num_jobs, int32_t dim) {
  return flat_workspace(job_rows, num_jobs, dim);
}

X2G_API int x2g_tiled_wgrad_flat_rows(const x2g_tiled_job* jobs, const int64_t* job_rows, int32_t num_jobs,
                                      int32_t dim, int flags, x2g_slab_job* slab_jobs, void* workspace,
                                      size_t workspace_bytes, void* stream) {
  return flat_launch(jobs, job_rows, num_jobs, dim, flags, slab_jobs, workspace, workspace_bytes, stream);
}

X2G_API size_t x2g_tiled_wgrad_workspace(int64_t rows, int32_t dim, int32_t num_jobs) {
  return x2g_chain_wgrad_workspace(rows, dim, num_jobs);
}

X2G_API int x2g_tiled_wgrad(const x2g_tiled_job* jobs, int32_t num_jobs, int64_t rows, int32_t dim, int flags,
                            void* workspace, size_t workspace_bytes, void* stream) {
  if (!jobs || num_jobs < 1 || num_jobs > X2G_CHAIN_MAX_STAGES || rows <= 0 || dim <= 0 ||
      (flags & ~(X2G_ACCUM_WGRAD | X2G_DEFER_SLAB_SUM)))
    return X2G_EINVAL;
  if (dim != kCD || rows * kCD * 4 >= (int64_t(1) << 31)) return X2G_EUNSUPPORTED;
  const size_t need = x2g_tiled_wgrad_workspace(rows, dim, num_jobs);
  if (!workspace || workspace_bytes < need) return X2G_EWORKSPACE;
  ChainWgradArgs a{};
  a.ntiles = (rows + 15) / 16;
  a.splits = chain_wgrad_splits(rows, dim, num_jobs);
  const size_t per = need / num_jobs;
  x2g_slab_job sj[X2G_CHAIN_MAX_STAGES];
  for (int j = 0; j < num_jobs; ++j) {
    const x2g_tiled_job& J = jobs[j];
    if (!J.dy_t || !J.x_t || !J.dw) return X2G_EINVAL;
    if (!al16(J.dy_t) || !al16(J.x_t)) return X2G_EUNSUPPORTED;
    a.in_t[j] = J.x_t;
    a.dz_t[j] = J.dy_t;
    a.part_w[j] = reinterpret_cast<float*>(static_cast<char*>(workspace) + per * j);
    a.part_b[j] = a.part_w[j] + static_cast<int64_t>(a.splits) * kCD * kCD;
    a.has_b[j] = J.db != nullptr;
    if (J.ld < 0 || (J.ld > 0 && (J.cols < 1 || J.cols > kCD || J.cols > J.ld))) return X2G_EINVAL;
    sj[j] = x2g_slab_job{a.part_w[j], J.db ? a.part_b[j] : nullptr, J.dw, J.db, kCD * kCD, J.db ? kCD : 0,
                         a.splits, J.ld, J.cols};
  }
  chain_wgrad_kernel<<<dim3(static_cast<unsigned>(a.splits), static_cast<unsigned>(num_jobs)), kCThreads, 0,
                       as_stream(stream)>>>(a);
  const int rc = last_launch_status();
  if (rc || (flags & X2G_DEFER_SLAB_SUM)) return rc;
  return x2g_slab_sum_batch(sj, num_jobs, (flags & X2G_ACCUM_WGRAD) ? 1 : 0, stream);
}
```

x2-gnn_amd/x2gnn/ops.py:

```python
from __future__ import annotations

import contextlib
import ctypes

import numpy as np
import torch

from . import _lib
from ._lib import call, ptr, stream_ptr

EDGE_NONE, EDGE_PER_TRIPLET, EDGE_PER_DST = 0, 1, 2


def rows_fit(rows, width):
    return int(rows) * int(width) * 4 < 2 ** 31


def _need_cuda(*ts):
    for t in ts:
        if t is not None and not t.is_cuda:
            raise RuntimeError("x2gnn device ops need GPU tensors (no CPU fallback by design)")


def _f32(t):
# ... 459 lines not shown
        prob = torch.empty(T, heads, dtype=torch.float32, device=dev)
        rho = torch.empty(E, heads, dtype=torch.float32, device=dev)
        gfold = torch.empty(E, 8, D, dtype=torch.float32, device=dev)
        st = stream_ptr()
        center, src_row = _center_rows(lg, mode, ctx.edge_row, D, channels)
        if sbf_p is not None or (center and _center_bwd_ok(lg, heads, s_rows=True)):
            want_edge = mode == EDGE_PER_DST and ctx.needs_input_grad[4]
            d_edge_atom = torch.empty(lg.N, D, dtype=torch.float32, device=dev) if want_edge else None
            g_work = torch.empty(2, T, heads, dtype=torch.float32, device=dev)
            call("x2g_sbf_attention_bwd_center", ptr(q), ptr(k), ptr(v), ptr(edge), ptr(src_row), mode, ptr(sproj),
                 ptr(sbf_p), ptr(b_sbf), ptr(ylm), ptr(lg.atom_rowptr), ptr(lg.edge_rev), ptr(lg.rev_trip), ptr(lg.center_order),
                 ptr(alpha), ptr(smax), ptr(sden), ptr(dout), lg.N, lg.max_degree, E, T, heads, channels, ptr(dq),
                 ptr(dk), ptr(dv), ptr(gfold), ptr(d_edge_atom), ptr(g_work), st)
            d_edge = None
            if want_edge:
                if ctx.defer_edge:
                    d_edge = keyed_row_sum_deferred(d_edge_atom, lg.atom_type, ctx.edge_shape[0], ctx.keyed_pending)
                else:
                    d_edge = keyed_row_sum(d_edge_atom, lg.atom_type, ctx.edge_shape[0])
            gw, gb = grad_sink(ctx.w_param), grad_sink(ctx.b_param)
            if gw is not None and gb is not None:
                dw, db = sbf_radial_wgrad(gfold, radial, dw_out=gw, db_out=gb)
            else:
                dw, db = sbf_radial_wgrad(gfold, radial)
            return dq, dk, dv, dout, d_edge, None, dw, db, None, None, None, None, None, None
        d_edge = torch.empty(E, D, dtype=torch.float32, device=dev) if mode == EDGE_PER_DST else None
        call("x2g_sbf_attention_bwd_dst_g", ptr(q), ptr(k), ptr(v), ptr(edge), ptr(ctx.edge_row), mode, ptr(sproj),
             ptr(lg.trip_rowptr), ptr(lg.trip_src), ptr(alpha), ptr(smax), ptr(sden), ptr(dout), E, T, heads, channels,
             ptr(dq), ptr(d_edge), ptr(g), ptr(prob), ptr(rho), st)
        src_rowptr, src_perm = lg.src_csr()
        rows = 0 if edge is None else edge.shape[0]
        src_row = lg.src_type if (ctx.edge_row is not None and ctx.edge_row is lg.dst_type) else None
        call("x2g_sbf_attention_bwd_src_fold", ptr(q), ptr(v), ptr(edge), ptr(ctx.edge_row), ptr(src_row), rows, mode,
             ptr(sproj), ptr(ylm), ptr(src_rowptr), ptr(src_perm), ptr(lg.src_dst), ptr(lg.trip_dst), ptr(prob),
             ptr(g), ptr(rho), ptr(dout), E, T, heads, channels, ptr(dk), ptr(dv), ptr(gfold), st)
        if not ctx.needs_input_grad[4]:
            d_edge = None
        elif mode == EDGE_PER_DST and ctx.edge_row is not None:
            if ctx.defer_edge:
                d_edge = keyed_row_sum_deferred(d_edge, ctx.edge_row, ctx.edge_shape[0], ctx.keyed_pending)
            else:
                d_edge = keyed_row_sum(d_edge, ctx.edge_row, ctx.edge_shape[0])
        gw, gb = grad_sink(ctx.w_param), grad_sink(ctx.b_param)
        if gw is not None and gb is not None:
            dw, db = sbf_radial_wgrad(gfold, radial, dw_out=gw, db_out=gb)
        else:
            dw, db = sbf_radial_wgrad(gfold, radial)
        return dq, dk, dv, dout, d_edge, None, dw, db, None, None, None, None, None, None


def sbf_radial_wgrad(gfold, radial, dw_out=None, db_out=None):
    E, _, D = gfold.shape
    accum = dw_out is not None
    if accum and db_out is None:
        raise ValueError("accumulating dW_sbf needs the bias-gradient buffer too")
    dw = dw_out if accum else torch.empty(D, 42, dtype=torch.float32, device=gfold.device)
    db = db_out if accum else torch.empty(D, dtype=torch.float32, device=gfold.device)
    lib = _lib.load()
    ws_bytes = int(lib.x2g_sbf_radial_wgrad_workspace(E, D))
    ws = torch.empty(max(ws_bytes, 1), dtype=torch.uint8, device=gfold.device)
    defer = accum and _defer() is not None and E > 0
    flags = (ACCUM_WGRAD if accum else 0) | (DEFER_SLAB_SUM if defer else 0)
    call("x2g_sbf_radial_wgrad", ptr(gfold), ptr(_f32(radial)), E, D, ptr(dw), ptr(db), flags, ptr(ws), ws_bytes,
         stream_ptr())
    if defer:
        _defer_job(ws, 0, int(lib.x2g_sbf_radial_wgrad_splits(E)), D * 42, D, dw, db)
    return (None, None) if accum else (dw, db)


class _EmbeddingTable(torch.autograd.Function):

    @staticmethod
    def forward(ctx, weight, z, max_norm, padding_idx, scale_grad):
        V, D = weight.shape
        if weight.dtype != torch.float32 or not weight.is_contiguous():
            raise ValueError("embedding weight must be contiguous fp32")
        zz = z if z.dtype == torch.int64 and z.is_contiguous() else z.to(torch.int64).contiguous()
        table = torch.empty_like(weight)
        counts = torch.empty(V, dtype=torch.float32, device=weight.device)
        call("x2g_embedding_table", ptr(weight), ptr(zz), zz.numel(), V, D, float(max_norm or 0.0), ptr(counts),
             ptr(table), stream_ptr())
        ctx.save_for_backward(counts)
        ctx.w_param, ctx.pad, ctx.scale = weight, (-1 if padding_idx is None else int(padding_idx)), bool(scale_grad)
        return table

    @staticmethod
    def backward(ctx, g):
        (counts,) = ctx.saved_tensors
        V, D = counts.shape[0], g.shape[1]
        sink = grad_sink(ctx.w_param)
        dw = sink if sink is not None else torch.empty(V, D, dtype=torch.float32, device=g.device)
        call("x2g_embedding_table_bwd", ptr(_f32(g)), ptr(counts) if ctx.scale else None, V, D, ctx.pad, ptr(dw),
             ACCUM_WGRAD if sink is not None else 0, stream_ptr())
        return (None if sink is not None else dw), None, None, None, None


def embedding_table(weight, z, max_norm, padding_idx, scale_grad_by_freq):
    _need_cuda(weight, z)
    return _EmbeddingTable.apply(weight, z, max_norm, padding_idx, scale_grad_by_freq)


class DenseFwdGroup(ctypes.Structure):
    _fields_ = [("x", ctypes.c_void_p), ("w", ctypes.c_void_p), ("b", ctypes.c_void_p), ("res", ctypes.c_void_p),
                ("y", ctypes.c_void_p), ("z", ctypes.c_void_p)]


class DenseBwdGroup(ctypes.Structure):
    _fields_ = [("dy", ctypes.c_void_p), ("z", ctypes.c_void_p), ("x", ctypes.c_void_p), ("w", ctypes.c_void_p),
                ("dx", ctypes.c_void_p), ("dx_add", ctypes.c_void_p), ("dw", ctypes.c_void_p),
                ("db", ctypes.c_void_p)]


class HeadGroup(ctypes.Structure):
    _fields_ = [("h", ctypes.c_void_p), ("w", ctypes.c_void_p), ("b", ctypes.c_void_p), ("dh", ctypes.c_void_p),
                ("dw", ctypes.c_void_p), ("db", ctypes.c_void_p)]


def _dp(t):
    return t.data_ptr() if t is not None else None


def _wgrad_targets(params, shapes, dev):
    sinks = [grad_sink(p) for p in params]
    if all(s is not None for s in sinks):
        return sinks, True
    return [torch.empty(sh, dtype=torch.float32, device=dev) for sh in shapes], False


class _ReadoutMLPs(torch.autograd.Function):

    @staticmethod
    def forward(ctx, G, pool, *args):
        feats, params = args[:G], args[G:]
        W1, B1, W2, B2, W3, B3 = (params[i::6] for i in range(6))
        R, D = feats[0].shape
        ctx.pool = pool
        dev = feats[0].device
        f32 = dict(dtype=torch.float32, device=dev)
        xs = [_f32(f) for f in feats]
        z1 = [torch.empty(R, D, **f32) for _ in range(G)]
        h2 = [torch.empty(R, D, **f32) for _ in range(G)]
        z2 = [torch.empty(R, D, **f32) for _ in range(G)]
        st = stream_ptr()
        ctx.chain = _readout_chain_ok(R, D, G, W1, B1, W2, B2)
        if ctx.chain:
            grad = _keeps(ctx)
            tf = int(_lib.load().x2g_chain_t_floats(R, D))
            WT = torch.empty(G, 2, D, D, **f32) if grad else None
            in_t = torch.empty(G, 2, tf, **f32) if grad else None

            def wt(g, i):
                return WT[g, i].data_ptr() if grad else None

            stages = [(ChainStage * 2)(ChainStage(_dp(W1[g]), _dp(B1[g]), _dp(z1[g]), None, wt(g, 0), CHAIN_SILU),
                                       ChainStage(_dp(W2[g]), _dp(B2[g]), _dp(z2[g]), _dp(h2[g]), wt(g, 1), CHAIN_SILU))
                      for g in range(G)]
            jobs = (ChainFwdJob * G)(*[ChainFwdJob(_dp(xs[g]), None, ctypes.addressof(stages[g]),
                                                   in_t[g].data_ptr() if grad else None) for g in range(G)])
            call("x2g_chain_fwd_batch", jobs, G, 2, R, D, st)
            heads = (HeadGroup * G)(*[HeadGroup(_dp(h2[g]), _dp(W3[g]), _dp(B3[g]), None, None, None)
                                      for g in range(G)])
            out = _head_fwd(heads, G, R, D, pool, f32, st)
            if grad:
                ctx.save_for_backward(*h2, *z1, *z2, WT, in_t)
            ctx.G, ctx.params = G, params
            return out
        h1 = [torch.empty(R, D, **f32) for _ in range(G)]
        for (src, w, b, y, z) in ((xs, W1, B1, h1, z1), (h1, W2, B2, h2, z2)):
            grp = (DenseFwdGroup * G)(*[DenseFwdGroup(_dp(src[g]), _dp(w[g]), _dp(b[g]), None, _dp(y[g]), _dp(z[g]))
                                        for g in range(G)])
            call("x2g_dense_fwd_batched", grp, G, R, D, D, ACT_SILU, st)
        heads = (HeadGroup * G)(*[HeadGroup(_dp(h2[g]), _dp(W3[g]), _dp(B3[g]), None, None, None) for g in range(G)])
        out = _head_fwd(heads, G, R, D, pool, f32, st)
        ctx.save_for_backward(*xs, *h1, *z1, *h2, *z2)
        ctx.G, ctx.params = G, params
        return out

    @staticmethod
    def backward(ctx, dout):
        G = ctx.G
        saved = ctx.saved_tensors
        if ctx.chain:
            h2, z1, z2 = (saved[i * G:(i + 1) * G] for i in range(3))
            WT, in_t = saved[3 * G], saved[3 * G + 1]
        else:
            xs, h1, z1, h2, z2 = (saved[i * G:(i + 1) * G] for i in range(5))
        W1, B1, W2, B2, W3, B3 = (ctx.params[i::6] for i in range(6))
        R, D = h2[0].shape
        dev = h2[0].device
        f32 = dict(dtype=torch.float32, device=dev)
        lib = _lib.load()
        st = stream_ptr()
        dout = _f32(dout.reshape(-1))
        dh2 = [torch.empty(R, D, **f32) for _ in range(G)]
        (dw3, db3), acc3 = _wgrad_pairs(W3, B3, dev)
        heads = (HeadGroup * G)(*[HeadGroup(_dp(h2[g]), _dp(W3[g]), None, _dp(dh2[g]), _dp(dw3[g]), _dp(db3[g]))
                                  for g in range(G)])
        ws_bytes = int(lib.x2g_readout_head_bwd_workspace(R, D, G))
        ws = torch.empty(max(ws_bytes, 1), dtype=torch.uint8, device=dev)
        defer = acc3 and _defer() is not None
        hflags = (ACCUM_WGRAD if acc3 else 0) | (DEFER_SLAB_SUM if defer else 0)
        if ctx.pool is not None:
            seg_rowptr, n_seg = ctx.pool
            call("x2g_readout_head_pool_bwd", ptr(dout), ptr(seg_rowptr), n_seg, heads, G, R, D, hflags, ptr(ws),
                 ws_bytes, st)
        else:
            call("x2g_readout_head_bwd", ptr(dout), heads, G, R, D, hflags, ptr(ws), ws_bytes, st)
        if defer:
            splits = int(lib.x2g_readout_head_bwd_splits(R))
            for g in range(G):
                _defer_job(ws, g * splits * (D + 1) * 4, splits, D, 1, dw3[g], db3[g])
        if ctx.chain:
            dfeat = [torch.empty(R, D, **f32) for _ in range(G)]
            dz_t = torch.empty_like(in_t)
            stages = [(ChainBwdStage * 2)(ChainBwdStage(_dp(W1[g]), WT[g, 0].data_ptr(), _dp(z1[g]), None, CHAIN_SILU),
                                          ChainBwdStage(_dp(W2[g]), WT[g, 1].data_ptr(), _dp(z2[g]), None, CHAIN_SILU))
                      for g in range(G)]
            jobs = (ChainBwdJob * G)(*[ChainBwdJob(_dp(dh2[g]), None, ctypes.addressof(stages[g]), _dp(dfeat[g]), None,
                                                   dz_t[g].data_ptr()) for g in range(G)])
            call("x2g_chain_bwd_batch", jobs, G, 2, R, D, st)
            pg = []
            for g in range(G):
                dws, dbs = chain_wgrad(in_t[g], dz_t[g], R, [W1[g], W2[g]], [B1[g], B2[g]])
                pg += [dws[0], dbs[0], dws[1], dbs[1]]
                pg += [None if acc3 else dw3[g].view_as(W3[g]), None if acc3 else db3[g]]
            return (None, None, *dfeat, *pg)
        grads = {}
        dy = dh2
        for (layer, x_in, z, W, B) in ((2, h1, z2, W2, B2), (1, xs, z1, W1, B1)):
            dx = [torch.empty(R, D, **f32) for _ in range(G)]
            (dw, db), acc = _wgrad_pairs(W, B, dev)
            grp = (DenseBwdGroup * G)(*[DenseBwdGroup(_dp(dy[g]), _dp(z[g]), _dp(x_in[g]), _dp(W[g]), _dp(dx[g]), None,
                                                      _dp(dw[g]), _dp(db[g])) for g in range(G)])
            wsz = int(lib.x2g_dense_bwd_workspace(R, D, D))
            ws = torch.empty(max(wsz * G, 1), dtype=torch.uint8, device=dev)
            defer = acc and _defer() is not None
            call("x2g_dense_bwd_batched", grp, G, R, D, D, ACT_SILU, (ACCUM_WGRAD if acc else 0) |
                 (DEFER_SLAB_SUM if defer else 0), ptr(ws), wsz * G, st)
            if defer:
                splits = int(lib.x2g_dense_bwd_splits(R, D, D))
                for g in range(G):
                    _defer_job(ws, g * wsz, splits, D * D, D, dw[g], db[g])
            grads[layer] = (None, None) if acc else (dw, db)
            dy = dx
        dfeat = dy
        pg = []
        for g in range(G):
            for (dw, db) in (grads[1], grads[2]):
                pg += [None if dw is None else dw[g], None if db is None else db[g]]
            pg += [None if acc3 else dw3[g].view_as(W3[g]), None if acc3 else db3[g]]
        return (None, None, *dfeat, *pg)


def _head_fwd(heads, G, R, D, pool, f32, st):
    if pool is None:
        out = torch.empty(R, 1, **f32)
        call("x2g_readout_head_fwd", heads, G, R, D, ptr(out), st)
        return out
    seg_rowptr, n_seg = pool
    out = torch.empty(n_seg, 1, **f32)
    call("x2g_readout_head_pool_fwd", heads, G, R, D, ptr(seg_rowptr), n_seg, ptr(out), st)
    return out


CHAIN_MAX_JOBS = 8


class ChainFwdJob(ctypes.Structure):
    _fields_ = [("x", ctypes.c_void_p), ("res_ext", ctypes.c_void_p), ("stages", ctypes.c_void_p),
                ("in_t", ctypes.c_void_p)]


class ChainBwdJob(ctypes.Structure):
    _fields_ = [("dy", ctypes.c_void_p), ("dy_add", ctypes.c_void_p), ("stages", ctypes.c_void_p),
                ("dx", ctypes.c_void_p), ("d_res_ext", ctypes.c_void_p), ("dz_t", ctypes.c_void_p)]


def _readout_chain_ok(R, D, G, *weights):
    if not _CHAIN or D != 128 or not 1 <= G <= CHAIN_MAX_JOBS or not rows_fit(R, 128):
        return False
    for ws in weights:
        for w in ws:
            if w is not None and (w.dtype != torch.float32 or not w.is_contiguous() or w.data_ptr() % 16):
                return False
    return all(tuple(w.shape) == (128, 128) for ws in (weights[0], weights[2]) for w in ws)


def _wgrad_pairs(Ws, Bs, dev):
    params = list(Ws) + list(Bs)
    bufs, acc = _wgrad_targets(params, [tuple(p.shape) for p in params], dev)
    n = len(Ws)
    return (bufs[:n], bufs[n:]), acc


def readout_mlps_supported(feats, mlps):
    from .layers import Linear as _Lin
    G = len(feats)
    if G < 1 or G > 8 or not all(f.is_cuda and f.dim() == 2 and f.shape == feats[0].shape for f in feats):
        return False
    R, D = feats[0].shape
    if D % 4 or D <= 8 or D > 128 or (D // 4) & (D // 4 - 1) or not rows_fit(R, 128):
        return False
    for m in mlps:
        mods = list(m)
        if len(mods) != 5 or not all(isinstance(mods[i], _Lin) for i in (0, 2, 4)):
            return False
        if not all(isinstance(mods[i], torch.nn.SiLU) for i in (1, 3)):
            return False
        if any(mods[i].bias is None for i in (0, 2, 4)):
            return False
        if tuple(mods[0].weight.shape) != (D, D) or tuple(mods[2].weight.shape) != (D, D):
            return False
        if tuple(mods[4].weight.shape) != (1, D):
            return False
    return True


def readout_mlps(feats, mlps, pool=None):
    params = []
    for m in mlps:
        mods = list(m)
        params += [mods[0].weight, mods[0].bias, mods[2].weight, mods[2].bias, mods[4].weight, mods[4].bias]
    if pool is not None:
        pool = (_i32(pool[0]), int(pool[1]))
    return _apply(_ReadoutMLPs, len(feats), pool, *feats, *params)


def keyed_row_sum(src, key, num_keys: int):
    _need_cuda(src, key)
    src = _f32(src)
    R, D = src.shape
    if num_keys > 16 or D % 4 or D > 256 or (D // 4) & (D // 4 - 1):
        onehot = torch.nn.functional.one_hot(key.long(), num_keys).to(torch.float32)
        return linear_wgrad(src, onehot, bias=False)[0].t().contiguous()
    out = torch.empty(num_keys, D, dtype=torch.float32, device=src.device)
    ws_bytes = int(_lib.load().x2g_keyed_row_sum_workspace(R, D, num_keys))
    ws = torch.empty(max(ws_bytes, 1), dtype=torch.uint8, device=src.device)
    call("x2g_keyed_row_sum", ptr(src), ptr(_i32(key)), R, D, num_keys, ptr(out), 0, ptr(ws), ws_bytes, stream_ptr())
    return out


_DEFER_KEYED = True
KEYED_MAX_JOBS = 8


def keyed_row_sum_deferred(src, key, num_keys: int, pending: list):
    src = _f32(src)
    R, D = src.shape
    if R == 0 or num_keys > 16 or D % 4 or D > 256 or (D // 4) & (D // 4 - 1):
        return keyed_row_sum(src, key, num_keys)
    out = torch.empty(num_keys, D, dtype=torch.float32, device=src.device)
    pending.append((src, _i32(key), int(num_keys), out))
    return out


def flush_keyed(pending: list):
    if not pending:
        return
    items = list(pending)
    pending.clear()
    groups = {}
    for src, key, nk, out in items:
        groups.setdefault((key.data_ptr(), tuple(src.shape), nk), []).append((src, key, nk, out))
    lib = _lib.load()
    for (_, (R, D), nk), items in groups.items():
        for j0 in range(0, len(items), KEYED_MAX_JOBS):
            part = items[j0:j0 + KEYED_MAX_JOBS]
            n = len(part)
            srcs = (ctypes.c_void_p * n)(*[it[0].data_ptr() for it in part])
            outs = (ctypes.c_void_p * n)(*[it[3].data_ptr() for it in part])
            wsb = int(lib.x2g_keyed_row_sum_batch_workspace(R, D, nk, n))
            ws = torch.empty(max(wsb, 1), dtype=torch.uint8, device=part[0][0].device)
            call("x2g_keyed_row_sum_batch", srcs, outs, n, ptr(part[0][1]), R, D, nk, 0, ptr(ws), wsb, stream_ptr())


INFER_TILE = 1 << 24
# ... 241 lines not shown

    def register(self):
        self.registered += 1
        return self

    def take(self, shape, device):
        first = self.buf is None
        if first:
            self.buf = torch.empty(shape, dtype=torch.float32, device=device)
        buf = self.buf
        self.used += 1
        if self.used >= self.registered:
            self.buf, self.used = None, 0
        return buf, first


def _fan_of(t):
    f = getattr(t, "_x2g_fanin", None) if t is not None else None
    return f.register() if f is not None else None


def linear_wgrad(dy, x, bias=True, dw_out=None, db_out=None):
    _need_cuda(dy, x)
    dy, x = _f32(dy), _f32(x)
    R, O = dy.shape
    I = x.shape[1]
    accum = dw_out is not None
    if accum and bias and db_out is None:
        raise ValueError("accumulating dW needs the bias-gradient buffer too")
    dw = dw_out if accum else torch.empty(O, I, dtype=torch.float32, device=dy.device)
    db = (db_out if accum else torch.empty(O, dtype=torch.float32, device=dy.device)) if bias else None
    ws_bytes = int(_lib.load().x2g_linear_wgrad_workspace(R, O, I))
    ws = torch.empty(max(ws_bytes, 1), dtype=torch.uint8, device=dy.device)
    defer = accum and _defer() is not None and R > 0
    flags = (ACCUM_WGRAD if accum else 0) | (DEFER_SLAB_SUM if defer else 0)
    call("x2g_linear_wgrad_ex", ptr(dy), ptr(x), R, O, I, ptr(dw), ptr(db), flags, ptr(ws), ws_bytes, stream_ptr())
    if defer:
        _defer_job(ws, 0, int(_lib.load().x2g_linear_wgrad_splits(R, O, I)), O * I, O, dw, db)
    return (None, None) if accum else (dw, db)


ACT_NONE, ACT_SILU = 0, 1


def _dense_fwd_raw(x2, w, b, act, r2=None, want_z=True):
    N, K = w.shape
    R = x2.shape[0]
    y = torch.empty(R, N, dtype=torch.float32, device=x2.device)
    z = torch.empty(R, N, dtype=torch.float32, device=x2.device) if (act != ACT_NONE and want_z) else None
    call("x2g_dense_fwd", ptr(x2), ptr(w), ptr(b), R, K, N, act, ptr(r2), ptr(y), ptr(z), stream_ptr())
    return y, z


def _dense_bwd_raw(gy2, z, act, x2, w, w_param, b_param, has_bias, need_dx, dx_add=None, dx_out=None):
    N, K = w.shape
    R = gy2.shape[0]
    dev = gy2.device
    dx = None
    if need_dx or dx_add is not None:
        dx = dx_out if dx_out is not None else torch.empty(R, K, dtype=torch.float32, device=dev)
    gw = grad_sink(w_param)
    gb = grad_sink(b_param) if has_bias else None
    accum = gw is not None and (gb is not None or not has_bias)
    if accum:
        dw, db = gw, gb
    else:
        dw = torch.empty(N, K, dtype=torch.float32, device=dev)
        db = torch.empty(N, dtype=torch.float32, device=dev) if has_bias else None
    lib = _lib.load()
    ws_bytes = int(lib.x2g_dense_bwd_workspace(R, K, N))
    ws = torch.empty(max(ws_bytes, 1), dtype=torch.uint8, device=dev)
    defer = accum and _defer() is not None and R > 0
    flags = (ACCUM_WGRAD if accum else 0) | (DEFER_SLAB_SUM if defer else 0)
    call("x2g_dense_bwd_ex", ptr(gy2), ptr(z), act, ptr(x2), ptr(w), R, K, N, ptr(dx), ptr(dx_add), ptr(dw), ptr(db),
         flags, ptr(ws), ws_bytes, stream_ptr())
    if defer:
        _defer_job(ws, lib.x2g_dense_bwd_slab_offset(R, K, N), int(lib.x2g_dense_bwd_splits(R, K, N)), N * K, N, dw,
                   db)
    if accum:
        return dx, None, None
    return dx, dw, db


class _DenseFn(torch.autograd.Function):

    @staticmethod
    def forward(ctx, x, weight, bias, res, act):
        N, K = weight.shape
        lead = x.shape[:-1]
        x2 = _f32(x.reshape(-1, K))
        w = _f32(weight)
        b = _f32(bias) if bias is not None else None
        r2 = _f32(res.reshape(-1, N)) if res is not None else None
        y, z = _dense_fwd_raw(x2, w, b, act, r2)
        ctx.save_for_backward(x2, w, z)
        ctx.act, ctx.has_bias, ctx.has_res, ctx.lead = act, bias is not None, res is not None, lead
        ctx.w_param, ctx.b_param = weight, bias
        return y.view(*lead, N)

    @staticmethod
    def backward(ctx, gy):
        x2, w, z = ctx.saved_tensors
        N, K = w.shape
        need_x = ctx.needs_input_grad[0]
        dx, dw, db = _dense_bwd_raw(_f32(gy.reshape(-1, N)), z, ctx.act, x2, w, ctx.w_param, ctx.b_param,
                                    ctx.has_bias, need_x)
        dres = gy if ctx.has_res else None
        dx = dx.view(*ctx.lead, K) if need_x else None
        return dx, dw, db, dres, None


class _ResidualFn(torch.autograd.Function):

    @staticmethod
    def forward(ctx, x, w0, b0, w1, b1):
        D = x.shape[-1]
        lead = x.shape[:-1]
        x2 = _f32(x.reshape(-1, D))
        W0, W1 = _f32(w0), _f32(w1)
        B0 = _f32(b0) if b0 is not None else None
        B1 = _f32(b1) if b1 is not None else None
        R = x2.shape[0]
        if W0.shape == (D, D) and W1.shape == (D, D) and D % 4 == 0 and 8 < D <= 128:
            f32 = dict(dtype=torch.float32, device=x2.device)
            h, z0, z1, y = (torch.empty(R, D, **f32) for _ in range(4))
            call("x2g_residual_fwd", ptr(x2), ptr(W0), ptr(B0), ptr(W1), ptr(B1), R, D, ptr(h), ptr(z0), ptr(z1),
                 ptr(y), stream_ptr())
        else:
            h, z0 = _dense_fwd_raw(x2, W0, B0, ACT_SILU)
            y, z1 = _dense_fwd_raw(h, W1, B1, ACT_SILU, r2=x2)
        ctx.save_for_backward(x2, h, z0, z1, W0, W1)
        ctx.params = (w0, b0, w1, b1)
        ctx.lead = lead
        return y.view(*lead, W1.shape[0])

    @staticmethod
    def backward(ctx, gy):
        x2, h, z0, z1, W0, W1 = ctx.saved_tensors
        w0, b0, w1, b1 = ctx.params
        gy2 = _f32(gy.reshape(-1, W1.shape[0]))
        dh, dw1, db1 = _dense_bwd_raw(gy2, z1, ACT_SILU, h, W1, w1, b1, b1 is not None, True)
        dx, dw0, db0 = _dense_bwd_raw(dh, z0, ACT_SILU, x2, W0, w0, b0, b0 is not None, True, dx_add=gy2)
        return dx.view(*ctx.lead, W0.shape[1]), dw0, db0, dw1, db1


def residual_layer(x, w0, b0, w1, b1):
    if not x.is_cuda:
        raise RuntimeError("x2gnn device ops need GPU tensors (no CPU fallback by design)")
    return _ResidualFn.apply(x, w0, b0, w1, b1)


CHAIN_SILU, CHAIN_HOLD, CHAIN_RES_HELD, CHAIN_RES_EXT = 1, 2, 4, 8
CHAIN_RES_ACCUM = 16
CHAIN_MAX_STAGES = 8


class ChainStage(ctypes.Structure):
    _fields_ = [("w", ctypes.c_void_p), ("b", ctypes.c_void_p), ("z", ctypes.c_void_p), ("y", ctypes.c_void_p),
                ("wt", ctypes.c_void_p), ("flags", ctypes.c_int32)]


class ChainBwdStage(ctypes.Structure):
    _fields_ = [("w", ctypes.c_void_p), ("wt", ctypes.c_void_p), ("z", ctypes.c_void_p), ("dz", ctypes.c_void_p),
                ("flags", ctypes.c_int32)]


class WgradJob(ctypes.Structure):
    _fields_ = [("dy", ctypes.c_void_p), ("x", ctypes.c_void_p), ("dw", ctypes.c_void_p), ("db", ctypes.c_void_p)]


def wgrad_batched(dys, xs, weights, biases):
    G = len(dys)
    R, D = dys[0].shape
    dev = dys[0].device
    params = list(weights) + [b for b in biases if b is not None]
    bufs, acc = _wgrad_targets(params, [tuple(p.shape) for p in params], dev)
    dws, rest = bufs[:G], iter(bufs[G:])
    dbs = [next(rest) if b is not None else None for b in biases]
    lib = _lib.load()
    ws_bytes = int(lib.x2g_wgrad_batched_workspace(R, D, G))
    ws = torch.empty(max(ws_bytes, 1), dtype=torch.uint8, device=dev)
    jobs = (WgradJob * G)(*[WgradJob(_dp(dys[g]), _dp(xs[g]), _dp(dws[g]), _dp(dbs[g])) for g in range(G)])
    defer = acc and _defer() is not None
    call("x2g_wgrad_batched", jobs, G, R, D, (ACCUM_WGRAD if acc else 0) | (DEFER_SLAB_SUM if defer else 0), ptr(ws),
         ws_bytes, stream_ptr())
    if defer:
        splits = int(lib.x2g_wgrad_batched_splits(R, D, G))
        per = ws_bytes // G
        for g in range(G):
            _defer_job(ws, g * per, splits, D * D, D, dws[g], dbs[g])
    if acc:
        return [None] * G, [None] * G
    return dws, dbs


def chain_wgrad(in_t, dz_t, R, weights, biases):
    n = len(weights)
    D = weights[0].shape[1]
    dev = in_t.device
    params = list(weights) + [b for b in biases if b is not None]
    bufs, acc = _wgrad_targets(params, [tuple(p.shape) for p in params], dev)
    dws, rest = bufs[:n], iter(bufs[n:])
    dbs = [next(rest) if b is not None else None for b in biases]
    d = _defer() if acc else None
    if d is not None:
        tf = in_t.shape[1]
        _queue_tiled(d, R, [TiledJob(dz_t.data_ptr() + 4 * g * tf, in_t.data_ptr() + 4 * g * tf, _dp(dws[g]), _dp(dbs[g]),
                                  0, 0) for g in range(n)], [in_t, dz_t])
        return [None] * n, [None] * n
    lib = _lib.load()
    ws_bytes = int(lib.x2g_chain_wgrad_workspace(R, D, n))
    ws = torch.empty(max(ws_bytes, 1), dtype=torch.uint8, device=dev)
    dw_arr = (ctypes.c_void_p * n)(*[_dp(t) for t in dws])
    db_arr = (ctypes.c_void_p * n)(*[_dp(t) for t in dbs])
    call("x2g_chain_wgrad", ptr(in_t), ptr(dz_t), n, R, D, dw_arr, db_arr, ACCUM_WGRAD if acc else 0, ptr(ws),
         ws_bytes, stream_ptr())
    if acc:
        return [None] * n, [None] * n
    return dws, dbs


class _ChainFn(torch.autograd.Function):

    @staticmethod
    def forward(ctx, x, res, flags, ln, *params):
        n = len(flags)
        ws, bs = params[0::2], params[1::2]
        x2 = _f32(x)
        R, D = x2.shape
        r2 = _f32(res) if res is not None else None
        f32 = dict(dtype=torch.float32, device=x2.device)
        grad = _keeps(ctx)
        zs = [torch.empty(R, D, **f32) if (flags[i] & CHAIN_SILU) and grad else None for i in range(n)]
        y = torch.empty(R, D, **f32)
        W = [_f32(w) for w in ws]
        B = [_f32(b) if b is not None else None for b in bs]
        tf = int(_lib.load().x2g_chain_t_floats(R, D))
        WT = torch.empty(n, D, D, **f32) if grad else None
        in_t = torch.empty(n, tf, **f32) if grad else None
        st = (ChainStage * n)(*[ChainStage(_dp(W[i]), _dp(B[i]), _dp(zs[i]), _dp(y) if i == n - 1 else None,
                                           None if WT is None else WT[i].data_ptr(), flags[i]) for i in range(n)])
        ctx.ln = ln is not None
        if ln is None:
            call("x2g_chain_fwd", ptr(x2), ptr(r2), st, n, R, D, ptr(in_t), stream_ptr())
            ln_saved = ()
        else:
            stats, rowptr, G, eps = ln
            xn = torch.empty(R, D, **f32) if grad else None
            rstd = torch.empty(G, **f32) if grad else None
            call("x2g_chain_fwd_ln", ptr(x2), ptr(stats), ptr(rowptr), G, float(eps), ptr(xn), None, ptr(rstd),
                 ptr(r2), st, n, R, D, ptr(in_t), stream_ptr())
            ln_saved = (xn, rstd, rowptr)
            ctx.ln_segments = G
        if grad:
            ctx.save_for_backward(*W, *[z if z is not None else x2 for z in zs], WT, in_t, *ln_saved)
        ctx.flags, ctx.params, ctx.has_res = tuple(flags), params, res is not None
        ctx.fan_res = _fan_of(res)
        return y

    @staticmethod
    def backward(ctx, gy):
        flags = ctx.flags
        n = len(flags)
        saved = ctx.saved_tensors
        W, zs, WT, in_t = saved[:n], saved[n:2 * n], saved[2 * n], saved[2 * n + 1]
        gy2 = _f32(gy)
        R, D = gy2.shape
        f32 = dict(dtype=torch.float32, device=gy2.device)
        dz_t = torch.empty_like(in_t)
        dx = torch.empty(R, D, **f32)
        dres, first = None, True
        if ctx.has_res and ctx.needs_input_grad[1]:
            if ctx.fan_res is not None:
                dres, first = ctx.fan_res.take((R, D), gy2.device)
            else:
                dres = torch.empty(R, D, **f32)
        bflags = [f | (CHAIN_RES_ACCUM if (f & CHAIN_RES_EXT) and not first else 0) for f in flags]
        st = (ChainBwdStage * n)(*[ChainBwdStage(_dp(W[i]), WT[i].data_ptr(),
                                                 _dp(zs[i]) if flags[i] & CHAIN_SILU else None, None, bflags[i])
                                   for i in range(n)])
        if not ctx.ln:
            call("x2g_chain_bwd", ptr(gy2), None, st, n, R, D, ptr(dx), ptr(dres), ptr(dz_t), stream_ptr())
        elif _LN_BWD_ROWS:
            xn, rstd, rowptr = saved[2 * n + 2:2 * n + 5]
            gst = torch.empty(R, 2, **f32)
            call("x2g_chain_bwd_ln", ptr(gy2), None, st, n, R, D, ptr(dx), ptr(dres), ptr(dz_t), ptr(xn), ptr(gst),
                 stream_ptr())
            dxp = torch.empty(R, D, **f32)
            call("x2g_graph_layernorm_bwd_rows", ptr(xn), ptr(dx), ptr(rstd), ptr(rowptr), ctx.ln_segments, D, ptr(gst),
                 ptr(dxp), stream_ptr())
            dx = dxp
        else:
            call("x2g_chain_bwd", ptr(gy2), None, st, n, R, D, ptr(dx), ptr(dres), ptr(dz_t), stream_ptr())
            xn, rstd, rowptr = saved[2 * n + 2:2 * n + 5]
            G = ctx.ln_segments
            dxp = torch.empty(R, D, **f32)
            wsb = int(_lib.load().x2g_graph_layernorm_bwd_workspace(G))
            lws = torch.empty(max(wsb, 1), dtype=torch.uint8, device=gy2.device)
            call("x2g_graph_layernorm_bwd_ex", ptr(xn), ptr(dx), ptr(rstd), ptr(rowptr), G, D, ptr(dxp), ptr(lws), wsb,
                 stream_ptr())
            dx = dxp
        ws, bs = ctx.params[0::2], ctx.params[1::2]
        dws, dbs = chain_wgrad(in_t, dz_t, R, ws, bs)
        grads = []
        for i in range(n):
            grads += [dws[i], dbs[i]]
        return (dx, dres if first else None, None, None, *grads)


def chain_supported(x, linears):
    if not x.is_cuda or x.dim() != 2 or x.shape[1] != 128 or not rows_fit(x.shape[0], 128):
        return False
    if len(linears) < 1 or len(linears) > CHAIN_MAX_STAGES:
        return False
    for m in linears:
        if tuple(m.weight.shape) != (128, 128) or m.weight.dtype != torch.float32 or m.weight.data_ptr() % 16:
            return False
        if m.bias is not None and m.bias.data_ptr() % 16:
            return False
    return True


_CHAIN = True


def row_chain(x, res, linears, flags, ln=None):
    params = []
    for m in linears:
        params += [m.weight, m.bias]
    if ln is not None:
        stats, rowptr, G, eps = ln
        ln = (_f32(stats), _i32(rowptr), int(G), float(eps))
    return _apply(_ChainFn, x, res, tuple(flags), ln, *params)


TABLE_MAX_STAGES = 8
_FAN_IN = True


class TableStage(ctypes.Structure):
    _fields_ = [("w", ctypes.c_void_p), ("b", ctypes.c_void_p), ("parent", ctypes.c_int32), ("act", ctypes.c_int32),
                ("z", ctypes.c_void_p), ("y", ctypes.c_void_p)]


class TableBwdStage(ctypes.Structure):
    _fields_ = [("w", ctypes.c_void_p), ("in_", ctypes.c_void_p), ("z", ctypes.c_void_p), ("dy", ctypes.c_void_p),
                ("dw", ctypes.c_void_p), ("db", ctypes.c_void_p), ("parent", ctypes.c_int32), ("act", ctypes.c_int32),
                ("accum", ctypes.c_int32)]


def table_chain_supported(x, linears):
    if not x.is_cuda or x.dim() != 2 or x.shape[1] != 128 or x.shape[0] > 16:
        return False
    if not 1 <= len(linears) <= TABLE_MAX_STAGES:
        return False
    for m in linears:
        if tuple(m.weight.shape) != (128, 128) or m.weight.dtype != torch.float32 or m.weight.data_ptr() % 16:
            return False
        if m.bias is not None and (m.bias.dtype != torch.float32 or m.bias.data_ptr() % 16):
            return False
    return True


class _TableChainFn(torch.autograd.Function):

    @staticmethod
    def forward(ctx, x, spec, pending, *params):
        n = len(spec)
        x2 = _f32(x).contiguous()
        R, D = x2.shape
        dev = x2.device
        ws = [_f32(p).contiguous() for p in params[0::2]]
        bs = [_f32(p).contiguous() if p is not None else None for p in params[1::2]]
        f32 = dict(dtype=torch.float32, device=dev)
        ys = [torch.empty(R, D, **f32) for _ in range(n)]
        zs = [torch.empty(R, D, **f32) if spec[s][1] == ACT_SILU else None for s in range(n)]
        st = (TableStage * n)(*[TableStage(_dp(ws[s]), _dp(bs[s]), spec[s][0], spec[s][1], _dp(zs[s]), _dp(ys[s]))
                                for s in range(n)])
        call("x2g_table_chain_fwd", ptr(x2), R, D, st, n, stream_ptr())
        ctx.save_for_backward(x2, *ws, *ys, *zs)
        ctx.spec, ctx.params, ctx.pending = spec, params, pending
        ctx.set_materialize_grads(False)
        return tuple(ys)

    @staticmethod
    def backward(ctx, *gys):
        flush_keyed(ctx.pending)
        spec, n = ctx.spec, len(ctx.spec)
        saved = ctx.saved_tensors
        x2, ws, ys, zs = saved[0], saved[1:1 + n], saved[1 + n:1 + 2 * n], saved[1 + 2 * n:1 + 3 * n]
        R, D = x2.shape
        dev = x2.device
        dys = [_f32(g).contiguous() if g is not None else None for g in gys]
        grads, stages = [], []
        for s in range(n):
            wp, bp = ctx.params[2 * s], ctx.params[2 * s + 1]
            gw = grad_sink(wp)
            gb = grad_sink(bp) if bp is not None else None
            accum = gw is not None and (bp is None or gb is not None)
            if accum:
                dw, db = gw, gb
                grads += [None, None]
            else:
                dw = torch.empty(D, D, dtype=torch.float32, device=dev)
                db = torch.empty(D, dtype=torch.float32, device=dev) if bp is not None else None
                grads += [dw, db]
            par, act = spec[s]
            src = x2 if par < 0 else ys[par]
            stages.append(TableBwdStage(_dp(ws[s]), _dp(src), _dp(zs[s]), _dp(dys[s]), _dp(dw), _dp(db), par, act,
                                        1 if accum else 0))
        dx = torch.empty(R, D, dtype=torch.float32, device=dev) if ctx.needs_input_grad[0] else None
        wsb = int(_lib.load().x2g_table_chain_bwd_workspace(n))
        ws = torch.empty(max(wsb, 16), dtype=torch.uint8, device=dev)
        call("x2g_table_chain_bwd_ex", (TableBwdStage * n)(*stages), n, R, D, ptr(dx), ptr(ws), wsb, stream_ptr())
        return (dx, None, None, *grads)


def table_chain(x, stages):
    params, spec = [], []
    for m, act, parent in stages:
        params += [m.weight, m.bias]
        spec.append((int(parent), int(act)))
    pending = []
    outs = _TableChainFn.apply(x, tuple(spec), pending, *params)
    for o in outs:
        o._x2g_keyed_pending = pending
    return outs


def featurize_supported(x, env, lin1, lin2):
    if not x.is_cuda or x.dim() != 2 or x.dtype != torch.float32 or x.requires_grad:
        return False
    R, K = x.shape
    if not (256 < K <= 384 and K % 2 == 0) or not rows_fit(R, 384):
        return False
    if env is not None and (env.numel() != R or env.requires_grad):
        return False
    if tuple(lin1.weight.shape) != (256, K) or tuple(lin2.weight.shape) != (128, 256):
        return False
    for p in (lin1.weight, lin1.bias, lin2.weight, lin2.bias):
        if p is not None and (p.dtype != torch.float32 or p.data_ptr() % 16):
            return False
    return True


class _FeaturizeFn(torch.autograd.Function):

    @staticmethod
    def forward(ctx, x, env, w1, b1, w2, b2):
        x2 = _f32(x)
        R, K = x2.shape
        dev = x2.device
        tf = int(_lib.load().x2g_chain_t_floats(R, 128))
        f32 = dict(dtype=torch.float32, device=dev)
        y = torch.empty(R, 128, **f32)
        grad = _keeps(ctx)
        xs_t, z1_t, y1_t, z2_t = ((torch.empty(max(n * tf, 1), **f32) for n in (3, 2, 2, 1)) if grad
                                  else (None, None, None, None))
        e = _f32(env.reshape(-1)) if env is not None else None
        W1, W2 = _f32(w1), _f32(w2)
        B1 = _f32(b1) if b1 is not None else None
        B2 = _f32(b2) if b2 is not None else None
        call("x2g_feat_fwd", ptr(x2), ptr(e), R, K, ptr(W1), ptr(B1), ptr(W2), ptr(B2), ptr(y), ptr(xs_t), ptr(z1_t),
             ptr(y1_t), ptr(z2_t), stream_ptr())
        if grad:
            ctx.save_for_backward(xs_t, z1_t, y1_t, z2_t, W2)
        ctx.R, ctx.K, ctx.tf = R, K, tf
        ctx.params = (w1, b1, w2, b2)
        return y

    @staticmethod
    def backward(ctx, gy):
        xs_t, z1_t, y1_t, z2_t, W2 = ctx.saved_tensors
        R, K, tf = ctx.R, ctx.K, ctx.tf
        dev = gy.device
        f32 = dict(dtype=torch.float32, device=dev)
        dz2_t, dz1_t = torch.empty(max(tf, 1), **f32), torch.empty(max(2 * tf, 1), **f32)
        call("x2g_feat_bwd", ptr(_f32(gy)), ptr(z2_t), ptr(z1_t), ptr(W2), R, ptr(dz2_t), ptr(dz1_t), stream_ptr())
        w1, b1, w2, b2 = ctx.params
        params = [p for p in (w1, b1, w2, b2) if p is not None]
        bufs, acc = _wgrad_targets(params, [tuple(p.shape) for p in params], dev)
        it = iter(bufs)
        dw1 = next(it)
        db1 = next(it) if b1 is not None else None
        dw2 = next(it)
        db2 = next(it) if b2 is not None else None
        fb = 4
        specs = []
        for o in range(2):
            for i in range(3):
                specs.append((dz1_t.data_ptr() + fb * o * tf, xs_t.data_ptr() + fb * i * tf,
                              dw1.data_ptr() + fb * (o * 128 * K + i * 128),
                              db1.data_ptr() + fb * o * 128 if (db1 is not None and i == 0) else None, K,
                              min(128, K - 128 * i)))
        for i in range(2):
            specs.append((dz2_t.data_ptr(), y1_t.data_ptr() + fb * i * tf, dw2.data_ptr() + fb * i * 128,
                          db2.data_ptr() if (db2 is not None and i == 0) else None, 256, 128))
        n = len(specs)
        d = _defer() if acc else None
        if d is not None:
            _queue_tiled(d, R, [TiledJob(*sp) for sp in specs], [dz1_t, dz2_t, xs_t, y1_t])
            return None, None, None, None, None, None
        lib = _lib.load()
        ws_bytes = int(lib.x2g_tiled_wgrad_workspace(R, 128, n))
        ws = torch.empty(max(ws_bytes, 1), dtype=torch.uint8, device=dev)
        jobs = (TiledJob * n)(*[TiledJob(*sp) for sp in specs])
        call("x2g_tiled_wgrad", jobs, n, R, 128, ACCUM_WGRAD if acc else 0, ptr(ws), ws_bytes, stream_ptr())
        if acc:
            return None, None, None, None, None, None
        return None, None, dw1, db1, dw2, db2


def featurize(x, env, lin1, lin2):
    return _apply(_FeaturizeFn, x, env, lin1.weight, lin1.bias, lin2.weight, lin2.bias)


class TiledJob(ctypes.Structure):
    _fields_ = [("dy_t", ctypes.c_void_p), ("x_t", ctypes.c_void_p), ("dw", ctypes.c_void_p), ("db", ctypes.c_void_p),
                ("ld", ctypes.c_int32), ("cols", ctypes.c_int32)]


class Proj(ctypes.Structure):
    _fields_ = [("w", ctypes.c_void_p), ("b", ctypes.c_void_p), ("out", ctypes.c_void_p), ("wt", ctypes.c_void_p)]


class ProjGrad(ctypes.Structure):
    _fields_ = [("g", ctypes.c_void_p), ("w", ctypes.c_void_p), ("wt", ctypes.c_void_p), ("g_t", ctypes.c_void_p)]


def tiled_wgrad(dy_ts, x_ts, R, weights, biases):
    n = len(weights)
    D = weights[0].shape[1]
    dev = dy_ts[0].device
    params = list(weights) + [b for b in biases if b is not None]
    bufs, acc = _wgrad_targets(params, [tuple(p.shape) for p in params], dev)
    dws, rest = bufs[:n], iter(bufs[n:])
    dbs = [next(rest) if b is not None else None for b in biases]
    d = _defer() if acc else None
    if d is not None:
        _queue_tiled(d, R, [TiledJob(_dp(dy_ts[g]), _dp(x_ts[g]), _dp(dws[g]), _dp(dbs[g]), 0, 0) for g in range(n)],
                     list(dy_ts) + list(x_ts))
        return [None] * n, [None] * n
    lib = _lib.load()
    ws_bytes = int(lib.x2g_tiled_wgrad_workspace(R, D, n))
    ws = torch.empty(max(ws_bytes, 1), dtype=torch.uint8, device=dev)
    jobs = (TiledJob * n)(*[TiledJob(_dp(dy_ts[g]), _dp(x_ts[g]), _dp(dws[g]), _dp(dbs[g])) for g in range(n)])
    call("x2g_tiled_wgrad", jobs, n, R, D, ACCUM_WGRAD if acc else 0, ptr(ws), ws_bytes, stream_ptr())
    if acc:
        return [None] * n, [None] * n
    return dws, dbs


def conv_proj_fused_supported(x, rbf, weights, biases):
    if not _CHAIN or not x.is_cuda or x.dim() != 2 or x.shape[1] != 128 or not rows_fit(x.shape[0], 128):
        return False
    if rbf.dim() != 2 or not 1 <= rbf.shape[1] <= 8 or rbf.shape[0] != x.shape[0]:
        return False
    for w in weights:
        if tuple(w.shape) != (128, 128) or w.dtype != torch.float32 or w.data_ptr() % 16:
            return False
    return all(b is None or b.data_ptr() % 16 == 0 for b in biases)


def _conv_proj_bwd_gate(grads, x2, rbf2, Wr, wr, dx, first_x, need_rbf, drbf_out, first_r):
    E, D = x2.shape
    RR = rbf2.shape[1]
    dev = x2.device
    drbf = drbf_out if drbf_out is not None else (
        torch.empty(E, RR, dtype=torch.float32, device=dev) if need_rbf else None)
    gw = grad_sink(wr)
    accum = gw is not None
    dw = gw if accum else torch.empty(D, RR, dtype=torch.float32, device=dev)
    lib = _lib.load()
    ws_bytes = int(lib.x2g_conv_proj_bwd_gate_workspace(E, RR))
    ws = torch.empty(max(ws_bytes, 1), dtype=torch.uint8, device=dev)
    defer = accum and _defer() is not None and E > 0
    flags = ((ACCUM_WGRAD if accum else 0) | (DEFER_SLAB_SUM if defer else 0)
             | (GATE_DRBF_ACCUM if (need_rbf and not first_r) else 0))
    call("x2g_conv_proj_bwd_gate", grads, E, D, ptr(x2), ptr(rbf2), RR, ptr(Wr), ptr(dx),
         None if first_x else ptr(dx), ptr(drbf), ptr(dw), flags, ptr(ws), ws_bytes, stream_ptr())
    if defer:
        _defer_job(ws, 0, int(lib.x2g_conv_proj_bwd_gate_splits(E)), D * RR, 0, dw, None)
    return dx, drbf, (None if accum else dw)


class _ConvProjFusedFn(torch.autograd.Function):

    @staticmethod
    def forward(ctx, x, rbf, wr, wq, bq, wk, bk, wv, bv, ws, bs):
        E, D = x.shape
        x2, rbf2, Wr = _f32(x), _f32(rbf), _f32(wr)
        W = [_f32(t) for t in (wq, wk, wv, ws)]
        B = [_f32(t) if t is not None else None for t in (bq, bk, bv, bs)]
        f32 = dict(dtype=torch.float32, device=x2.device)
        outs = [torch.empty(E, D, **f32) for _ in range(4)]
        grad = _keeps(ctx)
        lib = _lib.load()
        tf = int(lib.x2g_chain_t_floats(E, D))
        WT = torch.empty(4, D, D, **f32) if grad else None
        x_t = torch.empty(tf, **f32) if grad else None
        xs_t = torch.empty(tf, **f32) if grad else None
        proj = (Proj * 4)(*[Proj(_dp(W[i]), _dp(B[i]), _dp(outs[i]), None if WT is None else WT[i].data_ptr())
                            for i in range(4)])
        call("x2g_conv_proj_fwd", ptr(x2), ptr(rbf2), rbf2.shape[1], ptr(Wr), proj, E, D, ptr(x_t), ptr(xs_t),
             stream_ptr())
        if grad:
            ctx.save_for_backward(x2, rbf2, Wr, *W, WT, x_t, xs_t)
        ctx.params = (wr, wq, bq, wk, bk, wv, bv, ws, bs)
        ctx.fan_x, ctx.fan_r = _fan_of(x), _fan_of(rbf)
        return tuple(outs)

    @staticmethod
    def backward(ctx, gq, gk, gv, gskip):
        x2, rbf2, Wr, Wq, Wk, Wv, Ws, WT, x_t, xs_t = ctx.saved_tensors
        wr, wq, bq, wk, bk, wv, bv, ws, bs = ctx.params
        E, D = x2.shape
        f32 = dict(dtype=torch.float32, device=x2.device)
        g = [_f32(t) if t is not None else torch.zeros(E, D, **f32) for t in (gq, gk, gv, gskip)]
        tf = x_t.shape[0]
        g_t = torch.empty(4, tf, **f32)
        W = (Wq, Wk, Wv, Ws)
        grads = (ProjGrad * 4)(*[ProjGrad(_dp(g[i]), _dp(W[i]), WT[i].data_ptr(), g_t[i].data_ptr())
                                 for i in range(4)])
        first_x = first_r = True
        if ctx.fan_x is not None:
            dx, first_x = ctx.fan_x.take((E, D), x2.device)
        else:
            dx = torch.empty(E, D, **f32)
        need_rbf = ctx.needs_input_grad[1]
        drbf_out = None
        if need_rbf and ctx.fan_r is not None:
            drbf_out, first_r = ctx.fan_r.take(rbf2.shape, x2.device)
        gx, grbf, dwr = _conv_proj_bwd_gate(grads, x2, rbf2, Wr, wr, dx, first_x, need_rbf, drbf_out, first_r)
        gx = gx if first_x else None
        grbf = grbf if first_r else None
        dws, dbs = tiled_wgrad([g_t[0], g_t[1], g_t[2], g_t[3]], [x_t, xs_t, xs_t, x_t], E, [wq, wk, wv, ws],
                               [bq, bk, bv, bs])
        return (gx, (grbf if need_rbf else None), dwr, dws[0], dbs[0], dws[1], dbs[1], dws[2], dbs[2], dws[3],
                dbs[3])


class _ConvProjFn(torch.autograd.Function):

    @staticmethod
    def forward(ctx, x, rbf, wr, wq, bq, wk, bk, wv, bv, ws, bs):
        E, D = x.shape
        x2, rbf2 = _f32(x), _f32(rbf)
        Wr, Wq, Wk, Wv, Ws = (_f32(t) for t in (wr, wq, wk, wv, ws))
        Bq, Bk, Bv, Bs = (_f32(t) if t is not None else None for t in (bq, bk, bv, bs))
        if gate_supported(D, rbf2.shape[1]):
            rf = None
            xs = torch.empty_like(x2)
            call("x2g_rbf_gate_fwd", ptr(x2), ptr(rbf2), ptr(Wr), None, E, D, rbf2.shape[1], ptr(xs), stream_ptr())
        else:
            rf, _ = _dense_fwd_raw(rbf2, Wr, None, ACT_NONE)
            xs = x2 * rf
        q, k, v, skip = _projections4(x2, xs, (Wq, Bq), (Wk, Bk), (Wv, Bv), (Ws, Bs))
        ctx.save_for_backward(x2, rbf2, rf, xs, Wr, Wq, Wk, Wv, Ws)
        ctx.params = (wr, wq, bq, wk, bk, wv, bv, ws, bs)
        return q, k, v, skip

    @staticmethod
    def backward(ctx, gq, gk, gv, gskip):
        x2, rbf2, rf, xs, Wr, Wq, Wk, Wv, Ws = ctx.saved_tensors
        wr, wq, bq, wk, bk, wv, bv, ws, bs = ctx.params
        g = [_f32(t) if t is not None else torch.zeros_like(x2) for t in (gq, gk, gv, gskip)]
        gxs, dwk, dbk = _dense_bwd_raw(g[1], None, ACT_NONE, xs, Wk, wk, bk, bk is not None, True)
        gxs, dwv, dbv = _dense_bwd_raw(g[2], None, ACT_NONE, xs, Wv, wv, bv, bv is not None, True, dx_add=gxs,
                                       dx_out=gxs)
        need_rbf = ctx.needs_input_grad[1]
        if rf is None:
            gx, grbf, dwr, _ = _gate_bwd(gxs, None, x2, rbf2, Wr, None, wr, None, True, need_rbf)
        else:
            grf = gxs * x2
            gx = gxs * rf
        gx, dwq, dbq = _dense_bwd_raw(g[0], None, ACT_NONE, x2, Wq, wq, bq, bq is not None, True, dx_add=gx,
                                      dx_out=gx)
        gx, dws, dbs = _dense_bwd_raw(g[3], None, ACT_NONE, x2, Ws, ws, bs, bs is not None, True, dx_add=gx,
                                      dx_out=gx)
        if rf is not None:
            grbf, dwr, _ = _dense_bwd_raw(grf, None, ACT_NONE, rbf2, Wr, wr, None, False, need_rbf)
        return gx, (grbf if need_rbf else None), dwr, dwq, dbq, dwk, dbk, dwv, dbv, dws, dbs


def _projections4(x2, xs, pq, pk, pv, ps):
    R, K = x2.shape
    N = pq[0].shape[0]
    outs = [torch.empty(R, N, dtype=torch.float32, device=x2.device) for _ in range(4)]
    ok = (K % 4 == 0 and N % 4 == 0 and 8 < K <= 128 and N <= 128 and rows_fit(R, 128)
          and all(p[0].shape == pq[0].shape for p in (pk, pv, ps)))
    if ok and R > 0:
        srcs = (x2, xs, xs, x2)
        grp = (DenseFwdGroup * 4)(*[DenseFwdGroup(_dp(srcs[g]), _dp(p[0]), _dp(p[1]), None, _dp(outs[g]), None)
                                    for g, p in enumerate((pq, pk, pv, ps))])
        call("x2g_dense_fwd_batched", grp, 4, R, K, N, ACT_NONE, stream_ptr())
        return outs
    return [_dense_fwd_raw(src, p[0], p[1], ACT_NONE)[0] for src, p in zip((x2, xs, xs, x2), (pq, pk, pv, ps))]


def gate_supported(D, R):
    return D in (64, 128, 256) and 1 <= R <= 8


def _gate_bwd(g, owner, x, rbf, w, b, w_param, b_param, need_dx, need_rbf, dx_add=None, dx_out=None, drbf_out=None,
              drbf_acc=False):
    rows, D = x.shape
    R = rbf.shape[1]
    dev = x.device
    dx = dx_out if dx_out is not None else (torch.empty(rows, D, dtype=torch.float32, device=dev) if need_dx else None)
    drbf = drbf_out if drbf_out is not None else (
        torch.empty(rows, R, dtype=torch.float32, device=dev) if need_rbf else None)
    has_bias = b is not None
    gw, gb = grad_sink(w_param), (grad_sink(b_param) if has_bias else None)
    accum = gw is not None and (gb is not None or not has_bias)
    if accum:
        dw, db = gw, gb
    else:
        dw = torch.empty(D, R, dtype=torch.float32, device=dev)
        db = torch.empty(D, dtype=torch.float32, device=dev) if has_bias else None
    lib = _lib.load()
    ws_bytes = int(lib.x2g_rbf_gate_bwd_workspace(rows, D, R))
    ws = torch.empty(max(ws_bytes, 1), dtype=torch.uint8, device=dev)
    defer = accum and _defer() is not None and rows > 0
    flags = (ACCUM_WGRAD if accum else 0) | (DEFER_SLAB_SUM if defer else 0) | (GATE_DRBF_ACCUM if drbf_acc else 0)
    call("x2g_rbf_gate_bwd", ptr(g), ptr(owner), ptr(x), ptr(rbf), ptr(w), ptr(b), rows, D, R, ptr(dx), ptr(dx_add),
         ptr(drbf), ptr(dw), ptr(db), flags, ptr(ws), ws_bytes, stream_ptr())
    if defer:
        _defer_job(ws, 0, int(lib.x2g_rbf_gate_bwd_splits(rows)), D * R, D, dw, db)
    return dx, drbf, (None if accum else dw), (None if accum else db)


class _RbfPoolFn(torch.autograd.Function):

    @staticmethod
    def forward(ctx, x, rbf, w, b, owner, rowptr, n_seg):
        x2, rbf2, W = _f32(x), _f32(rbf), _f32(w)
        B = _f32(b) if b is not None else None
        D, R = x2.shape[1], rbf2.shape[1]
        out = torch.empty(n_seg, D, dtype=torch.float32, device=x2.device)
        call("x2g_rbf_pool_fwd", ptr(x2), ptr(rbf2), ptr(W), ptr(B), ptr(rowptr), n_seg, D, R, ptr(out), stream_ptr())
        ctx.save_for_backward(x2, rbf2, W, B)
        ctx.owner, ctx.params = owner, (w, b)
        ctx.fan_x, ctx.fan_r = _fan_of(x), _fan_of(rbf)
        return out

    @staticmethod
    def backward(ctx, gp):
        x2, rbf2, W, B = ctx.saved_tensors
        w, b = ctx.params
        need_x, need_r = ctx.needs_input_grad[0], ctx.needs_input_grad[1]
        dev = x2.device
        dx_out = drbf_out = None
        first_x = first_r = True
        if need_x and ctx.fan_x is not None:
            dx_out, first_x = ctx.fan_x.take(x2.shape, dev)
        if need_r and ctx.fan_r is not None:
            drbf_out, first_r = ctx.fan_r.take(rbf2.shape, dev)
        dx, drbf, dw, db = _gate_bwd(_f32(gp), ctx.owner, x2, rbf2, W, B, w, b, need_x, need_r,
                                     dx_add=None if first_x else dx_out, dx_out=dx_out, drbf_out=drbf_out,
                                     drbf_acc=not first_r)
        return (dx if first_x else None), (drbf if first_r else None), dw, db, None, None, None


def _addr(t):
    return None if t is None else t.data_ptr()


class GateJob(ctypes.Structure):
    _fields_ = [("x", ctypes.c_void_p), ("w", ctypes.c_void_p), ("b", ctypes.c_void_p), ("out", ctypes.c_void_p),
                ("g", ctypes.c_void_p), ("dx", ctypes.c_void_p), ("dx_add", ctypes.c_void_p), ("dw", ctypes.c_void_p),
                ("db", ctypes.c_void_p)]


GATE_MAX_JOBS = 8
_POOL_BATCH = True


class _RbfPoolBatchFn(torch.autograd.Function):

    @staticmethod
    def forward(ctx, n, rbf, owner, rowptr, n_seg, *tensors):
        xs, ws, bs = tensors[:n], tensors[n:2 * n], tensors[2 * n:]
        rbf2 = _f32(rbf)
        x2 = [_f32(x) for x in xs]
        W = [_f32(w) for w in ws]
        B = [_f32(b) if b is not None else None for b in bs]
        D, R = x2[0].shape[1], rbf2.shape[1]
        outs = [torch.empty(n_seg, D, dtype=torch.float32, device=rbf2.device) for _ in range(n)]
        jobs = (GateJob * n)(*[GateJob(x2[j].data_ptr(), W[j].data_ptr(), _addr(B[j]), outs[j].data_ptr(), None, None,
                                       None, None, None) for j in range(n)])
# ... 342 lines not shown
```

Before: 58200 molecules/s.

## Let tiled weight-grad kernel read row-major inputs to skip transposed copies

Adds row-major layout variants to the tiled weight-gradient kernel, using a swizzled LDS indexing scheme and templated dispatch. Forward chain and conv projection kernels can now skip writing transposed copies of the first-stage input and of the output gradients, reading the original row-major tensors in the backward pass instead. This removes transposed-copy stores and buffers in the forward and backward kernels. In exchange, the wgrad LDS reads become strided scalar gathers, which may add bank conflicts, and extra tensors are kept alive for backward.

```diff
diff --git a/include/x2g.h b/include/x2g.h
--- a/include/x2g.h
+++ b/include/x2g.h
@@ -406,6 +406,7 @@
 #define X2G_CHAIN_RES_HELD 4
 #define X2G_CHAIN_RES_EXT 8
 #define X2G_CHAIN_RES_ACCUM 16
+#define X2G_CHAIN_IN0_ROWMAJOR 32
 
 typedef struct {
   const float* w;
@@ -508,7 +509,11 @@
   float* db;
   int32_t ld;
   int32_t cols;
+  int32_t layout;
+  int32_t pad_;
 } x2g_tiled_job;
+#define X2G_TILED_DY_ROWMAJOR 1
+#define X2G_TILED_X_ROWMAJOR 2
 
 #define X2G_TILED_MAX_JOBS 64
 size_t x2g_tiled_wgrad_flat_workspace(int64_t rows, int32_t dim, int32_t num_jobs);
diff --git a/x2-gnn_amd/csrc/chain.hip b/x2-gnn_amd/csrc/chain.hip
--- a/x2-gnn_amd/csrc/chain.hip
+++ b/x2-gnn_amd/csrc/chain.hip
@@ -554,7 +554,7 @@
 #pragma unroll
     for (int rb = 0; rb < RB; ++rb) held[rb] = zero4();
     __syncthreads();
-    if (a.in_t) {
+    if (a.in_t && !(a.st[0].flags & X2G_CHAIN_IN0_ROWMAJOR)) {
       f4 xs[RB];
 #pragma unroll
       for (int rb = 0; rb < RB; ++rb) xs[rb] = img0[ipos(16 * rb + rl, 4 * w + g)];
@@ -938,34 +938,51 @@
   }
 }
 
-template <bool SPREAD, int WT>
+__device__ __forceinline__ int rpos(int r, int f) { return 128 * r + 4 * ((f >> 2) ^ (r & 12)) + (f & 3); }
+
+template <bool SPREAD, int WT, bool DR, bool XR>
 __device__ __forceinline__ void tiled_segment2(const float* __restrict__ dz, const float* __restrict__ xin, int64_t t0,
-                                               int64_t t1, bool has_b, float* __restrict__ slab,
+                                               int64_t t1, int64_t rows, bool has_b, float* __restrict__ slab,
                                                float* __restrict__ slab_b, f4 (*D0)[512], f4 (*X0)[512],
-                                               f4 (*D1)[512], f4 (*X1)[512]) {
+                                               f4 (*D1)[512], f4 (*X1)[512], float* __restrict__ bred) {
   const int tid = threadIdx.x, lane = tid & 63, w = tid >> 6;
   const int rl = lane & 15, g = lane >> 4;
   const int nsteps = static_cast<int>((t1 - t0 + WT - 1) / WT);
   const int P = 64 * w + lane;
-  const int src_chunk = (P >> 2) * 4 + ((P & 3) ^ (((P >> 5) & 1) * 3));
+  const int chunk_t = (P >> 2) * 4 + ((P & 3) ^ (((P >> 5) & 1) * 3));
+  const int chunk_r = (P & ~31) | ((P & 31) ^ ((P >> 5) & 12));
+  const int d_chunk = DR ? chunk_r : chunk_t, x_chunk = XR ? chunk_r : chunk_t;
   const int64_t nt = t1 - t0;
   const int nbytes = static_cast<int>(nt * 8192 < 0x7fffffff ? nt * 8192 : 0x7fffffff);
-  const rsrc_t dr = __builtin_amdgcn_make_buffer_rsrc(const_cast<float*>(dz + t0 * 2048), static_cast<short>(0), nbytes,
-                                                      0x00020000);
-  const rsrc_t xr = __builtin_amdgcn_make_buffer_rsrc(const_cast<float*>(xin + t0 * 2048), static_cast<short>(0), nbytes,
-                                                      0x00020000);
+  const int64_t rend = t1 * 16 < rows ? t1 * 16 : rows;
+  const int64_t rb64 = (rend - t0 * 16) * (kCD * 4);
+  const int rbytes = static_cast<int>(rb64 < 0x7fffffff ? rb64 : 0x7fffffff);
+  const rsrc_t dr = __builtin_amdgcn_make_buffer_rsrc(const_cast<float*>(dz + t0 * 2048), static_cast<short>(0),
+                                                      DR ? rbytes : nbytes, 0x00020000);
+  const rsrc_t xr = __builtin_amdgcn_make_buffer_rsrc(const_cast<float*>(xin + t0 * 2048), static_cast<short>(0),
+                                                      XR ? rbytes : nbytes, 0x00020000);
   auto issue = [&](int step, f4 (*Dd)[512], f4 (*Xd)[512]) {
 #pragma unroll
     for (int k = 0; k < WT; ++k) {
       int tt = step * WT + k;
       tt = tt < nt ? tt : 0;
-      const int vo = tt * 8192 + 16 * src_chunk;
-      __builtin_amdgcn_raw_ptr_buffer_load_lds(dr, (__attribute__((address_space(3))) void*)(&Dd[k][64 * w]), 16, vo, 0,
-                                               0, 0);
-      __builtin_amdgcn_raw_ptr_buffer_load_lds(xr, (__attribute__((address_space(3))) void*)(&Xd[k][64 * w]), 16, vo, 0,
-                                               0, 0);
+      __builtin_amdgcn_raw_ptr_buffer_load_lds(dr, (__attribute__((address_space(3))) void*)(&Dd[k][64 * w]), 16,
+                                               tt * 8192 + 16 * d_chunk, 0, 0, 0);
+      __builtin_amdgcn_raw_ptr_buffer_load_lds(xr, (__attribute__((address_space(3))) void*)(&Xd[k][64 * w]), 16,
+                                               tt * 8192 + 16 * x_chunk, 0, 0, 0);
     }
   };
+  auto quad = [&](const f4* im, bool rowmajor, int f, int q) {
+    if (!rowmajor) return im[tpos(f, q)];
+    const float* fm = reinterpret_cast<const float*>(im) + rpos(4 * q, f);
+    f4 v;
+#pragma unroll
+    for (int e = 0; e < 4; ++e) v[e] = fm[128 * e];
+    return v;
+  };
+  int xb[4];
+#pragma unroll
+  for (int j = 0; j < 4; ++j) xb[j] = rpos(4 * g, 16 * j + rl);
   f4 acc[8];
 #pragma unroll
   for (int bk = 0; bk < 8; ++bk) acc[bk] = zero4();
@@ -978,22 +995,30 @@
 #pragma unroll
     for (int k = 0; k < WT; ++k) {
       if (t0 + static_cast<int64_t>(i) * WT + k >= t1) break;
-      const f4 av = Dc[k][tpos(16 * w + rl, g)];
+      const f4 av = quad(Dc[k], DR, 16 * w + rl, g);
       f4 bv[8];
-#pragma unroll
-      for (int bk = 0; bk < 8; ++bk) bv[bk] = Xc[k][tpos(16 * bk + rl, g)];
+      if (XR) {
+        const float* fm = reinterpret_cast<const float*>(Xc[k]);
+#pragma unroll
+        for (int bk = 0; bk < 8; ++bk)
+#pragma unroll
+          for (int e = 0; e < 4; ++e) bv[bk][e] = fm[xb[bk & 3] + 64 * (bk >> 2) + 128 * e];
+      } else {
+#pragma unroll
+        for (int bk = 0; bk < 8; ++bk) bv[bk] = Xc[k][tpos(16 * bk + rl, g)];
+      }
 #pragma unroll
       for (int e = 0; e < 4; ++e)
 #pragma unroll
         for (int bk = 0; bk < 8; ++bk) acc[bk] = __builtin_amdgcn_mfma_f32_16x16x4f32(av[e], bv[bk][e], acc[bk], 0, 0, 0);
       if (SPREAD && has_b) {
-        const f4 v = Dc[k][tpos(tid & (kCD - 1), tid >> 7)];
+        const f4 v = quad(Dc[k], DR, tid & (kCD - 1), tid >> 7);
         bsum += (v[0] + v[1]) + (v[2] + v[3]);
       }
       if (!SPREAD && tid < 128) {
 #pragma unroll
         for (int q = 0; q < 4; ++q) {
-          const f4 v = Dc[k][tpos(tid, q)];
+          const f4 v = quad(Dc[k], DR, tid, q);
           bsum += (v[0] + v[1]) + (v[2] + v[3]);
         }
       }
@@ -1012,7 +1037,6 @@
     for (int e = 0; e < 4; ++e) slab[(16 * w + 4 * g + e) * kCD + 16 * bk + rl] = acc[bk][e];
   if (!SPREAD && has_b && tid < 128) slab_b[tid] = bsum;
   if (SPREAD && has_b) {
-    __shared__ float bred[4 * kCD];
     bred[tid] = bsum;
     __syncthreads();
     if (tid < kCD) slab_b[tid] = ((bred[tid] + bred[kCD + tid]) + bred[2 * kCD + tid]) + bred[3 * kCD + tid];
@@ -1035,6 +1059,8 @@
   float* slab_b[X2G_TILED_MAX_JOBS];
   int wg_lo[X2G_TILED_MAX_JOBS];
   int has_b[X2G_TILED_MAX_JOBS];
+  int layout[X2G_TILED_MAX_JOBS];
+  int rows[X2G_TILED_MAX_JOBS];
   int64_t tile0[X2G_TILED_MAX_JOBS + 1];
   int64_t total;
   int njobs;
@@ -1047,6 +1073,7 @@
   __shared__ f4 X0[WT][512];
   __shared__ f4 D1[WT][512];
   __shared__ f4 X1[WT][512];
+  __shared__ float bred[4 * kCD];
   const int64_t G = gridDim.x, i = blockIdx.x;
   const int64_t lo = i * a.total / G, hi = (i + 1) * a.total / G;
   int j0 = 0;
@@ -1057,8 +1084,19 @@
     if (s0 >= s1) continue;
     __syncthreads();
     const int64_t k = i - a.wg_lo[j];
-    tiled_segment2<SPREAD, WT>(a.dz_t[j], a.in_t[j], s0 - a.tile0[j], s1 - a.tile0[j], a.has_b[j] != 0,
-                               a.slab_w[j] + k * kCD * kCD, a.slab_b[j] + k * kCD, D0, X0, D1, X1);
+    auto seg = [&](auto dr, auto xr) {
+      tiled_segment2<SPREAD, WT, decltype(dr)::value, decltype(xr)::value>(
+          a.dz_t[j], a.in_t[j], s0 - a.tile0[j], s1 - a.tile0[j], a.rows[j], a.has_b[j] != 0,
+          a.slab_w[j] + k * kCD * kCD, a.slab_b[j] + k * kCD, D0, X0, D1, X1, bred);
+    };
+    using T_ = std::false_type;
+    using R_ = std::true_type;
+    switch (a.layout[j]) {
+      case 0: seg(T_{}, T_{}); break;
+      case X2G_TILED_DY_ROWMAJOR: seg(R_{}, T_{}); break;
+      case X2G_TILED_X_ROWMAJOR: seg(T_{}, R_{}); break;
+      default: seg(R_{}, R_{}); break;
+    }
   }
 }
 
@@ -1192,7 +1230,7 @@
 };
 
 
-template <int NJ, bool TW>
+template <int NJ, bool TW, bool TC>
 __global__ void __launch_bounds__(kCThreads, 2) conv_proj_bwd_gate_kernel(const ProjBwdGateArgs a) {
   constexpr int RB = kGateRB;
   constexpr int kImg = RB * 16 * 32;
@@ -1220,6 +1258,7 @@
       load_slice<true>(a.gr[p].w, w, rl, g, dst);
   };
   auto t_copy = [&](int p, const f4* im, int r0, int nrows) {
+    if (!TC) return;
     f4 v[RB];
 #pragma unroll
     for (int rb = 0; rb < RB; ++rb) v[rb] = im[ipos(16 * rb + rl, 4 * w + g)];
@@ -1235,8 +1274,9 @@
   const rsrc_t bo = rsrc_n(a.drbf, a.R * a.RR * 4, a.drbf != nullptr && a.drbf_acc);
   static_assert(RB * 16 * NJ <= kCThreads && RB * 16 * kRbfMax <= kCThreads, "one srbf / drbf element per thread");
   constexpr int kWL = TW ? 8 : 32;
-  constexpr int kKVWait = 3 * RB + 2 * kWL < 63 ? 3 * RB + 2 * kWL : 63;
-  constexpr int kQSWait = 2 * RB + 2 * kWL < 63 ? 2 * RB + 2 * kWL : 63;
+  constexpr int kTS = TC ? 2 * RB : 0;
+  constexpr int kKVWait = kTS + RB + 2 * kWL < 63 ? kTS + RB + 2 * kWL : 63;
+  constexpr int kQSWait = kTS + 2 * kWL < 63 ? kTS + 2 * kWL : 63;
   if (nk > 0) {
     int r0, nrows;
     chunk(0, r0, nrows);
@@ -1279,6 +1319,7 @@
       const int r = tid / NJ, j = tid % NJ;
       rbv = bload1(rr, (tid < RB * 16 * NJ && r < nrows && j < a.RR) ? 4 * ((r0 + r) * a.RR + j) : kOOB, 0);
     }
+    if (!TC) asm volatile("" ::: "memory");
     t_copy(1, img_k, r0, nrows);
     t_copy(2, img_v, r0, nrows);
     f4 acc1[RB];
@@ -1386,7 +1427,9 @@
   for (int s = 0; s < n_stages; ++s) {
     const x2g_chain_stage& S = stages[s];
     if (!S.w || (s == n_stages - 1 && !S.y)) return X2G_EINVAL;
-    if (S.flags & ~(X2G_CHAIN_SILU | X2G_CHAIN_HOLD | X2G_CHAIN_RES_HELD | X2G_CHAIN_RES_EXT)) return X2G_EINVAL;
+    if (S.flags & ~(X2G_CHAIN_SILU | X2G_CHAIN_HOLD | X2G_CHAIN_RES_HELD | X2G_CHAIN_RES_EXT |
+                    (s == 0 ? X2G_CHAIN_IN0_ROWMAJOR : 0)))
+      return X2G_EINVAL;
     if ((S.flags & X2G_CHAIN_RES_EXT) && (S.flags & (X2G_CHAIN_HOLD | X2G_CHAIN_RES_HELD))) return X2G_EINVAL;
     if (S.flags & X2G_CHAIN_RES_EXT) held = 0;
     if (S.flags & X2G_CHAIN_HOLD) held = 1;
@@ -1732,16 +1775,27 @@
   a.R = rows;
   const unsigned grid = proj_grid(rows);
   const bool tw = grads[0].wt && grads[1].wt && grads[2].wt && grads[3].wt;
-  if (rbf_dim <= 6) {
+  const bool tc = grads[0].g_t || grads[1].g_t || grads[2].g_t || grads[3].g_t;
+  auto launch = [&](auto nj, auto tw_, auto tc_) {
+    conv_proj_bwd_gate_kernel<decltype(nj)::value, decltype(tw_)::value, decltype(tc_)::value>
+        <<<grid, kCThreads, 0, st>>>(a);
+  };
+  auto pick_tc = [&](auto nj, auto tw_) {
+    if (tc)
+      launch(nj, tw_, std::true_type{});
+    else
+      launch(nj, tw_, std::false_type{});
+  };
+  auto pick_tw = [&](auto nj) {
     if (tw)
-      conv_proj_bwd_gate_kernel<6, true><<<grid, kCThreads, 0, st>>>(a);
+      pick_tc(nj, std::true_type{});
     else
-      conv_proj_bwd_gate_kernel<6, false><<<grid, kCThreads, 0, st>>>(a);
-  } else if (tw) {
-    conv_proj_bwd_gate_kernel<8, true><<<grid, kCThreads, 0, st>>>(a);
-  } else {
-    conv_proj_bwd_gate_kernel<8, false><<<grid, kCThreads, 0, st>>>(a);
-  }
+      pick_tc(nj, std::false_type{});
+  };
+  if (rbf_dim <= 6)
+    pick_tw(std::integral_constant<int, 6>{});
+  else
+    pick_tw(std::integral_constant<int, 8>{});
   const int rc = last_launch_status();
   if (rc || (flags & X2G_DEFER_SLAB_SUM)) return rc;
   x2g_slab_job sj{a.part_w, nullptr, dw_rbf, nullptr, static_cast<int64_t>(kCD) * rbf_dim, 0,
@@ -1812,6 +1866,9 @@
     if (!J.dy_t || !J.x_t || !J.dw) return X2G_EINVAL;
     if (!al16(J.dy_t) || !al16(J.x_t)) return X2G_EUNSUPPORTED;
     if (J.ld < 0 || (J.ld > 0 && (J.cols < 1 || J.cols > kCD || J.cols > J.ld))) return X2G_EINVAL;
+    if (J.layout & ~(X2G_TILED_DY_ROWMAJOR | X2G_TILED_X_ROWMAJOR)) return X2G_EINVAL;
+    a.layout[j] = J.layout;
+    a.rows[j] = static_cast<int>(rows[j]);
     int lo, n;
     flat_span(a.tile0[j], a.tile0[j + 1], a.total, G, lo, n);
     a.in_t[j] = J.x_t;
@@ -1880,6 +1937,7 @@
     const x2g_tiled_job& J = jobs[j];
     if (!J.dy_t || !J.x_t || !J.dw) return X2G_EINVAL;
     if (!al16(J.dy_t) || !al16(J.x_t)) return X2G_EUNSUPPORTED;
+    if (J.layout) return X2G_EUNSUPPORTED;
     a.in_t[j] = J.x_t;
     a.dz_t[j] = J.dy_t;
     a.part_w[j] = reinterpret_cast<float*>(static_cast<char*>(workspace) + per * j);
diff --git a/x2-gnn_amd/x2gnn/ops.py b/x2-gnn_amd/x2gnn/ops.py
--- a/x2-gnn_amd/x2gnn/ops.py
+++ b/x2-gnn_amd/x2gnn/ops.py
@@ -635,7 +635,10 @@
             def wt(g, i):
                 return WT[g, i].data_ptr() if grad else None
 
-            stages = [(ChainStage * 2)(ChainStage(_dp(W1[g]), _dp(B1[g]), _dp(z1[g]), None, wt(g, 0), CHAIN_SILU),
+            ctx.rm0 = WGRAD_X_ROWMAJOR and grad and all(grad_sink(p) is not None
+                                                        for p in (*W1, *B1, *W2, *B2) if p is not None)
+            f0 = CHAIN_SILU | (CHAIN_IN0_ROWMAJOR if ctx.rm0 else 0)
+            stages = [(ChainStage * 2)(ChainStage(_dp(W1[g]), _dp(B1[g]), _dp(z1[g]), None, wt(g, 0), f0),
                                        ChainStage(_dp(W2[g]), _dp(B2[g]), _dp(z2[g]), _dp(h2[g]), wt(g, 1), CHAIN_SILU))
                       for g in range(G)]
             jobs = (ChainFwdJob * G)(*[ChainFwdJob(_dp(xs[g]), None, ctypes.addressof(stages[g]),
@@ -645,7 +648,7 @@
                                       for g in range(G)])
             out = _head_fwd(heads, G, R, D, pool, f32, st)
             if grad:
-                ctx.save_for_backward(*h2, *z1, *z2, WT, in_t)
+                ctx.save_for_backward(*h2, *z1, *z2, WT, in_t, *(xs if ctx.rm0 else ()))
             ctx.G, ctx.params = G, params
             return out
         h1 = [torch.empty(R, D, **f32) for _ in range(G)]
@@ -704,7 +707,8 @@
             call("x2g_chain_bwd_batch", jobs, G, 2, R, D, st)
             pg = []
             for g in range(G):
-                dws, dbs = chain_wgrad(in_t[g], dz_t[g], R, [W1[g], W2[g]], [B1[g], B2[g]])
+                dws, dbs = chain_wgrad(in_t[g], dz_t[g], R, [W1[g], W2[g]], [B1[g], B2[g]],
+                                       x0=saved[3 * G + 2 + g] if ctx.rm0 else None)
                 pg += [dws[0], dbs[0], dws[1], dbs[1]]
                 pg += [None if acc3 else dw3[g].view_as(W3[g]), None if acc3 else db3[g]]
             return (None, None, *dfeat, *pg)
@@ -1252,6 +1256,7 @@
 
 CHAIN_SILU, CHAIN_HOLD, CHAIN_RES_HELD, CHAIN_RES_EXT = 1, 2, 4, 8
 CHAIN_RES_ACCUM = 16
+CHAIN_IN0_ROWMAJOR = 32
 CHAIN_MAX_STAGES = 8
 
 
@@ -1294,7 +1299,7 @@
     return dws, dbs
 
 
-def chain_wgrad(in_t, dz_t, R, weights, biases):
+def chain_wgrad(in_t, dz_t, R, weights, biases, x0=None):
     n = len(weights)
     D = weights[0].shape[1]
     dev = in_t.device
@@ -1303,11 +1308,19 @@
     dws, rest = bufs[:n], iter(bufs[n:])
     dbs = [next(rest) if b is not None else None for b in biases]
     d = _defer() if acc else None
-    if d is not None:
+    if d is not None or x0 is not None:
         tf = in_t.shape[1]
-        _queue_tiled(d, R, [TiledJob(dz_t.data_ptr() + 4 * g * tf, in_t.data_ptr() + 4 * g * tf, _dp(dws[g]), _dp(dbs[g]),
-                                  0, 0) for g in range(n)], [in_t, dz_t])
-        return [None] * n, [None] * n
+        jobs = [TiledJob(dz_t.data_ptr() + 4 * g * tf, in_t.data_ptr() + 4 * g * tf, _dp(dws[g]), _dp(dbs[g]), 0, 0)
+                for g in range(n)]
+        if x0 is not None:
+            jobs[0] = TiledJob(dz_t.data_ptr(), x0.data_ptr(), _dp(dws[0]), _dp(dbs[0]), 0, 0, TILED_X_ROWMAJOR)
+        if d is not None:
+            _queue_tiled(d, R, jobs, [in_t, dz_t] + ([x0] if x0 is not None else []))
+            return [None] * n, [None] * n
+        _tiled_now(R, jobs, acc, dev)
+        if acc:
+            return [None] * n, [None] * n
+        return dws, dbs
     lib = _lib.load()
     ws_bytes = int(lib.x2g_chain_wgrad_workspace(R, D, n))
     ws = torch.empty(max(ws_bytes, 1), dtype=torch.uint8, device=dev)
@@ -1338,8 +1351,10 @@
         tf = int(_lib.load().x2g_chain_t_floats(R, D))
         WT = torch.empty(n, D, D, **f32) if grad else None
         in_t = torch.empty(n, tf, **f32) if grad else None
+        ctx.rm0 = WGRAD_X_ROWMAJOR and grad and all(grad_sink(p) is not None for p in params if p is not None)
+        fl = [flags[i] | (CHAIN_IN0_ROWMAJOR if ctx.rm0 and i == 0 else 0) for i in range(n)]
         st = (ChainStage * n)(*[ChainStage(_dp(W[i]), _dp(B[i]), _dp(zs[i]), _dp(y) if i == n - 1 else None,
-                                           None if WT is None else WT[i].data_ptr(), flags[i]) for i in range(n)])
+                                           None if WT is None else WT[i].data_ptr(), fl[i]) for i in range(n)])
         ctx.ln = ln is not None
         if ln is None:
             call("x2g_chain_fwd", ptr(x2), ptr(r2), st, n, R, D, ptr(in_t), stream_ptr())
@@ -1353,7 +1368,8 @@
             ln_saved = (xn, rstd, rowptr)
             ctx.ln_segments = G
         if grad:
-            ctx.save_for_backward(*W, *[z if z is not None else x2 for z in zs], WT, in_t, *ln_saved)
+            ctx.save_for_backward(*W, *[z if z is not None else x2 for z in zs], WT, in_t, *ln_saved,
+                                  *((x2,) if ctx.rm0 and ln is None else ()))
         ctx.flags, ctx.params, ctx.has_res = tuple(flags), params, res is not None
         ctx.fan_res = _fan_of(res)
         return y
@@ -1401,7 +1417,7 @@
                  stream_ptr())
             dx = dxp
         ws, bs = ctx.params[0::2], ctx.params[1::2]
-        dws, dbs = chain_wgrad(in_t, dz_t, R, ws, bs)
+        dws, dbs = chain_wgrad(in_t, dz_t, R, ws, bs, x0=saved[2 * n + 2] if ctx.rm0 else None)
         grads = []
         for i in range(n):
             grads += [dws[i], dbs[i]]
@@ -1617,7 +1633,21 @@
 
 class TiledJob(ctypes.Structure):
     _fields_ = [("dy_t", ctypes.c_void_p), ("x_t", ctypes.c_void_p), ("dw", ctypes.c_void_p), ("db", ctypes.c_void_p),
-                ("ld", ctypes.c_int32), ("cols", ctypes.c_int32)]
+                ("ld", ctypes.c_int32), ("cols", ctypes.c_int32), ("layout", ctypes.c_int32), ("pad_", ctypes.c_int32)]
+
+
+TILED_DY_ROWMAJOR, TILED_X_ROWMAJOR = 1, 2
+
+WGRAD_X_ROWMAJOR = True
+
+
+def _tiled_now(R, jobs, acc, dev):
+    lib = _lib.load()
+    n = len(jobs)
+    ws_bytes = int(lib.x2g_tiled_wgrad_flat_workspace(R, 128, n))
+    ws = torch.empty(max(ws_bytes, 1), dtype=torch.uint8, device=dev)
+    call("x2g_tiled_wgrad_flat", (TiledJob * n)(*jobs), n, R, 128, ACCUM_WGRAD if acc else 0, None, ptr(ws), ws_bytes,
+         stream_ptr())
 
 
 class Proj(ctypes.Structure):
@@ -1628,7 +1658,7 @@
     _fields_ = [("g", ctypes.c_void_p), ("w", ctypes.c_void_p), ("wt", ctypes.c_void_p), ("g_t", ctypes.c_void_p)]
 
 
-def tiled_wgrad(dy_ts, x_ts, R, weights, biases):
+def tiled_wgrad(dy_ts, x_ts, R, weights, biases, layouts=None):
     n = len(weights)
     D = weights[0].shape[1]
     dev = dy_ts[0].device
@@ -1637,10 +1667,16 @@
     dws, rest = bufs[:n], iter(bufs[n:])
     dbs = [next(rest) if b is not None else None for b in biases]
     d = _defer() if acc else None
-    if d is not None:
-        _queue_tiled(d, R, [TiledJob(_dp(dy_ts[g]), _dp(x_ts[g]), _dp(dws[g]), _dp(dbs[g]), 0, 0) for g in range(n)],
-                     list(dy_ts) + list(x_ts))
-        return [None] * n, [None] * n
+    lay = layouts if layouts is not None else [0] * n
+    if d is not None or any(lay):
+        jobs = [TiledJob(_dp(dy_ts[g]), _dp(x_ts[g]), _dp(dws[g]), _dp(dbs[g]), 0, 0, lay[g]) for g in range(n)]
+        if d is not None:
+            _queue_tiled(d, R, jobs, list(dy_ts) + list(x_ts))
+            return [None] * n, [None] * n
+        _tiled_now(R, jobs, acc, dev)
+        if acc:
+            return [None] * n, [None] * n
+        return dws, dbs
     lib = _lib.load()
     ws_bytes = int(lib.x2g_tiled_wgrad_workspace(R, D, n))
     ws = torch.empty(max(ws_bytes, 1), dtype=torch.uint8, device=dev)
@@ -1698,30 +1734,27 @@
         lib = _lib.load()
         tf = int(lib.x2g_chain_t_floats(E, D))
         WT = torch.empty(4, D, D, **f32) if grad else None
-        x_t = torch.empty(tf, **f32) if grad else None
         xs_t = torch.empty(tf, **f32) if grad else None
+        x_t = torch.empty(tf, **f32) if grad and not WGRAD_X_ROWMAJOR else None
         proj = (Proj * 4)(*[Proj(_dp(W[i]), _dp(B[i]), _dp(outs[i]), None if WT is None else WT[i].data_ptr())
                             for i in range(4)])
         call("x2g_conv_proj_fwd", ptr(x2), ptr(rbf2), rbf2.shape[1], ptr(Wr), proj, E, D, ptr(x_t), ptr(xs_t),
              stream_ptr())
         if grad:
-            ctx.save_for_backward(x2, rbf2, Wr, *W, WT, x_t, xs_t)
+            ctx.save_for_backward(x2, rbf2, Wr, *W, WT, xs_t, x_t)
         ctx.params = (wr, wq, bq, wk, bk, wv, bv, ws, bs)
         ctx.fan_x, ctx.fan_r = _fan_of(x), _fan_of(rbf)
         return tuple(outs)
 
     @staticmethod
     def backward(ctx, gq, gk, gv, gskip):
-        x2, rbf2, Wr, Wq, Wk, Wv, Ws, WT, x_t, xs_t = ctx.saved_tensors
+        x2, rbf2, Wr, Wq, Wk, Wv, Ws, WT, xs_t, x_t = ctx.saved_tensors
         wr, wq, bq, wk, bk, wv, bv, ws, bs = ctx.params
         E, D = x2.shape
         f32 = dict(dtype=torch.float32, device=x2.device)
         g = [_f32(t) if t is not None else torch.zeros(E, D, **f32) for t in (gq, gk, gv, gskip)]
-        tf = x_t.shape[0]
-        g_t = torch.empty(4, tf, **f32)
         W = (Wq, Wk, Wv, Ws)
-        grads = (ProjGrad * 4)(*[ProjGrad(_dp(g[i]), _dp(W[i]), WT[i].data_ptr(), g_t[i].data_ptr())
-                                 for i in range(4)])
+        grads = (ProjGrad * 4)(*[ProjGrad(_dp(g[i]), _dp(W[i]), WT[i].data_ptr(), None) for i in range(4)])
         first_x = first_r = True
         if ctx.fan_x is not None:
             dx, first_x = ctx.fan_x.take((E, D), x2.device)
@@ -1734,8 +1767,10 @@
         gx, grbf, dwr = _conv_proj_bwd_gate(grads, x2, rbf2, Wr, wr, dx, first_x, need_rbf, drbf_out, first_r)
         gx = gx if first_x else None
         grbf = grbf if first_r else None
-        dws, dbs = tiled_wgrad([g_t[0], g_t[1], g_t[2], g_t[3]], [x_t, xs_t, xs_t, x_t], E, [wq, wk, wv, ws],
-                               [bq, bk, bv, bs])
+        xo = x2 if x_t is None else x_t
+        lx = TILED_DY_ROWMAJOR | (TILED_X_ROWMAJOR if x_t is None else 0)
+        dws, dbs = tiled_wgrad(g, [xo, xs_t, xs_t, xo], E, [wq, wk, wv, ws], [bq, bk, bv, bs],
+                               layouts=[lx, TILED_DY_ROWMAJOR, TILED_DY_ROWMAJOR, lx])
         return (gx, (grbf if need_rbf else None), dwr, dws[0], dbs[0], dws[1], dbs[1], dws[2], dbs[2], dws[3],
                 dbs[3])
 
```

New measurement: 59220 molecules/s (median of 6 runs). +1.7%, better.
